# trevor-m/cuda-pathtrace

Hardware: AMD Instinct MI355X
Metric: Msamples/s, 9-sphere Cornell box 1024x1024x1024spp (higher is better)
Workload: dtype f32+f64

## Files before the change

### cuda-pathtrace_amd/__init__.py

```python
import contextlib
import ctypes
import os

import numpy as np

_HERE = os.path.dirname(os.path.abspath(__file__))
LIB_PATH = os.environ.get("PT_LIB_OVERRIDE") or os.path.join(_HERE, "libptcore.so")
LAB_LIB_PATH = os.path.join(_HERE, "libptcore_lab.so")
INCLUDE_DIR = os.path.join(os.path.dirname(_HERE), "include")

if not os.path.exists(LIB_PATH):
    raise ImportError(
        f"{LIB_PATH} is missing: build it with `make -C cuda-pathtrace_amd/csrc` "
        "(or __graft_entry__.build()); there is no fallback implementation"
    )

RNG_XORWOW = 0
RNG_PHILOX = 1
CHANNELS = 14

SPHERE_DTYPE = np.dtype([("radius", "<f4"), ("pos", "<f4", 3), ("emission", "<f4", 3), ("color", "<f4", 3)])
assert SPHERE_DTYPE.itemsize == 40


# ... 129 lines not shown
    "pt_filter_run_frames": (ctypes.c_int, [_vp, ctypes.c_int, _vp, ctypes.c_size_t, _vp, ctypes.c_size_t, ctypes.c_int, _fp]),
    "pt_temporal_opts_default": (None, [_vp]),
    "pt_temporal_create": (ctypes.c_int, [ctypes.c_int, ctypes.c_int, _vp, ctypes.POINTER(_vp)]),
    "pt_temporal_destroy": (ctypes.c_int, [_vp]),
    "pt_temporal_reset": (ctypes.c_int, [_vp]),
    "pt_temporal_workspace_bytes": (ctypes.c_int, [_vp, ctypes.POINTER(ctypes.c_uint64)]),
    "pt_temporal_camera": (ctypes.c_int, [_fp, _fp]),
    "pt_temporal_antilag_opts_default": (None, [_vp]),
    "pt_temporal_antilag_check": (ctypes.c_int, [_vp, ctypes.c_float]),
    "pt_temporal_set_antilag": (ctypes.c_int, [_vp, _vp]),
    "pt_temporal_fast": (ctypes.c_int, [_vp, _vp, _vp]),
    "pt_temporal_enqueue": (ctypes.c_int, [_vp, _vp, ctypes.c_int, _fp, _fp, _vp, _vp]),
    "pt_temporal_run": (ctypes.c_int, [_vp, _vp, ctypes.c_int, _fp, _fp, _vp, _fp]),
    "pt_temporal_enqueue_frames": (ctypes.c_int, [_vp, ctypes.c_int, _vp, ctypes.c_size_t, _fp, _fp, ctypes.c_int, _vp, _vp]),
    "pt_temporal_run_frames": (ctypes.c_int, [_vp, ctypes.c_int, _vp, ctypes.c_size_t, _fp, _fp, ctypes.c_int, _vp, _fp]),
    "pt_temporal_scene_check": (ctypes.c_int, [_vp, _vp, ctypes.c_int, _fp, _fp]),
    "pt_temporal_motion": (ctypes.c_int, [_vp, _vp, _vp, ctypes.c_int, _fp, _fp, _vp, _vp]),
    "pt_temporal_enqueue_motion": (ctypes.c_int, [_vp, _vp, ctypes.c_int, _fp, _fp, _vp, _vp, _vp]),
    "pt_temporal_run_motion": (ctypes.c_int, [_vp, _vp, ctypes.c_int, _fp, _fp, _vp, _vp, _fp]),
    "pt_temporal_enqueue_scene": (ctypes.c_int, [_vp, _vp, ctypes.c_int, _fp, _fp, _vp, ctypes.c_int, _vp, _vp]),
    "pt_temporal_run_scene": (ctypes.c_int, [_vp, _vp, ctypes.c_int, _fp, _fp, _vp, ctypes.c_int, _vp, _fp]),
    "pt_temporal_enqueue_frames_scenes": (ctypes.c_int, [_vp, ctypes.c_int, _vp, ctypes.c_size_t, _fp, _fp, _vp, ctypes.c_int, ctypes.c_int, _vp, _vp]),
    "pt_temporal_run_frames_scenes": (ctypes.c_int, [_vp, ctypes.c_int, _vp, ctypes.c_size_t, _fp, _fp, _vp, ctypes.c_int, ctypes.c_int, _vp, _fp]),
    "pt_tonemap_opts_default": (None, [_vp]),
    "pt_tonemap_create": (ctypes.c_int, [ctypes.c_int, ctypes.c_int, _vp, ctypes.POINTER(_vp)]),
    "pt_tonemap_destroy": (ctypes.c_int, [_vp]),
    "pt_tonemap_reset": (ctypes.c_int, [_vp]),
    "pt_tonemap_workspace_bytes": (ctypes.c_int, [_vp, ctypes.POINTER(ctypes.c_uint64)]),
    "pt_tonemap_reserve_frames": (ctypes.c_int, [_vp, ctypes.c_int]),
    "pt_tonemap_srgb_table": (ctypes.c_int, [_fp]),
    "pt_tonemap_enqueue": (ctypes.c_int, [_vp, _vp, ctypes.c_int, _vp, _vp]),
    "pt_tonemap_run": (ctypes.c_int, [_vp, _vp, ctypes.c_int, _vp, _fp]),
    "pt_tonemap_enqueue_frames": (ctypes.c_int, [_vp, ctypes.c_int, _vp, ctypes.c_size_t, ctypes.c_int, _vp, ctypes.c_size_t, _vp]),
    "pt_tonemap_run_frames": (ctypes.c_int, [_vp, ctypes.c_int, _vp, ctypes.c_size_t, ctypes.c_int, _vp, ctypes.c_size_t, _fp]),
    "pt_tonemap_exposure": (ctypes.c_int, [_vp, _fp]),
    "pt_compare_opts_default": (None, [_vp]),
    "pt_compare_create": (ctypes.c_int, [ctypes.c_int, ctypes.c_int, _vp, ctypes.POINTER(_vp)]),
    "pt_compare_destroy": (ctypes.c_int, [_vp]),
    "pt_compare_workspace_bytes": (ctypes.c_int, [_vp, ctypes.POINTER(ctypes.c_uint64)]),
    "pt_compare_reserve_frames": (ctypes.c_int, [_vp, ctypes.c_int]),
    "pt_compare_ssim_weights": (ctypes.c_int, [_fp]),
    "pt_compare_enqueue": (ctypes.c_int, [_vp, _vp, ctypes.c_int, _vp, ctypes.c_int, _vp, _vp]),
    "pt_compare_run": (ctypes.c_int, [_vp, _vp, ctypes.c_int, _vp, ctypes.c_int, _vp, _fp]),
    "pt_compare_enqueue_frames": (ctypes.c_int, [_vp, ctypes.c_int, _vp, ctypes.c_size_t, ctypes.c_int, _vp, ctypes.c_size_t, ctypes.c_int, _vp,
                                                 ctypes.c_size_t, _vp]),
    "pt_compare_run_frames": (ctypes.c_int, [_vp, ctypes.c_int, _vp, ctypes.c_size_t, ctypes.c_int, _vp, ctypes.c_size_t, ctypes.c_int, _vp,
                                             ctypes.c_size_t, _fp]),
    "pt_compare_result": (ctypes.c_int, [_vp, ctypes.c_int, _vp]),
    "pt_patches_opts_default": (None, [_vp]),
    "pt_patches_create": (ctypes.c_int, [ctypes.c_int, ctypes.c_int, _vp, ctypes.POINTER(_vp)]),
    "pt_patches_destroy": (ctypes.c_int, [_vp]),
    "pt_patches_workspace_bytes": (ctypes.c_int, [_vp, ctypes.POINTER(ctypes.c_uint64)]),
    "pt_patches_prepare": (ctypes.c_int, [_vp, _vp, _vp]),
    "pt_patches_score": (ctypes.c_int, [_vp, _vp, ctypes.c_int, _vp, _vp]),
    "pt_patches_result": (ctypes.c_int, [_vp, ctypes.c_int, _vp]),
    "pt_patches_gather": (ctypes.c_int, [_vp, _vp, _vp, ctypes.c_int, ctypes.c_int, _vp, _vp, _vp, _vp]),
    "pt_patches_run_prepare": (ctypes.c_int, [_vp, _vp, _fp]),
    "pt_patches_run_score": (ctypes.c_int, [_vp, _vp, ctypes.c_int, _vp, _fp]),
    "pt_patches_run_gather": (ctypes.c_int, [_vp, _vp, _vp, ctypes.c_int, ctypes.c_int, _vp, _vp, _vp, _fp]),
    "pt_progressive_create": (ctypes.c_int, [_vp, ctypes.POINTER(_vp)]),
    "pt_progressive_reset": (ctypes.c_int, [_vp]),
    "pt_progressive_enqueue": (ctypes.c_int, [_vp, ctypes.c_int, _vp, _vp, ctypes.c_int, _fp, _fp, _vp]),
    "pt_progressive_render": (ctypes.c_int, [_vp, ctypes.c_int, _vp, _vp, ctypes.c_int, _fp, _fp, _fp]),
    "pt_progressive_samples": (ctypes.c_int, [_vp, ctypes.POINTER(ctypes.c_int64)]),
    "pt_progressive_variant": (ctypes.c_int, [_vp, ctypes.c_int, ctypes.POINTER(ctypes.c_int)]),
    "pt_progressive_destroy": (ctypes.c_int, [_vp]),
    "pt_progressive_set_adaptive": (ctypes.c_int, [_vp, _vp]),
    "pt_progressive_active": (ctypes.c_int, [_vp, ctypes.POINTER(ctypes.c_int64)]),
    "pt_progressive_counts": (ctypes.c_int, [_vp, _vp, _vp]),
}
LAB_ABI = {
    "pt_debug_unary_map": (ctypes.c_int, [ctypes.c_int, _vp, _vp, ctypes.c_size_t]),
    "pt_debug_unary_compare": (ctypes.c_int, [ctypes.c_int, ctypes.c_int, ctypes.c_uint32, ctypes.c_uint64,
                                              ctypes.POINTER(ctypes.c_uint64), ctypes.POINTER(ctypes.c_uint32)]),
    "pt_debug_div_compare": (ctypes.c_int, [ctypes.c_uint32, ctypes.c_uint32, ctypes.c_uint32, ctypes.c_uint64,
                                            ctypes.POINTER(ctypes.c_uint64), ctypes.POINTER(ctypes.c_uint32),
                                            ctypes.POINTER(ctypes.c_uint32)]),
    "pt_debug_grid_header": (ctypes.c_int, [_vp, ctypes.c_int, ctypes.POINTER(ctypes.c_uint32)]),
    "pt_debug_grid_image": (ctypes.c_int, [_vp, ctypes.c_int, _fp, ctypes.c_int, ctypes.POINTER(ctypes.c_uint32), ctypes.c_size_t,
                                           ctypes.POINTER(ctypes.c_uint64)]),
    "pt_debug_policy_ms": (ctypes.c_int, [ctypes.c_int, ctypes.c_int, ctypes.c_double, ctypes.c_int, ctypes.c_int, ctypes.POINTER(ctypes.c_double)]),
    "pt_debug_policy_choice": (ctypes.c_int, [ctypes.c_int, ctypes.c_double, ctypes.c_int, ctypes.c_int, ctypes.c_int, ctypes.c_int, ctypes.POINTER(ctypes.c_int)]),
    "pt_debug_renderer_batch_launches": (ctypes.c_int, [_vp, ctypes.POINTER(ctypes.c_uint32)]),
    "pt_debug_kernel_builds": (ctypes.c_int, [ctypes.c_int, ctypes.POINTER(ctypes.c_int), ctypes.POINTER(ctypes.c_int32)]),
    "pt_debug_variant_row": (ctypes.c_int, [ctypes.c_int, ctypes.POINTER(ctypes.c_int), ctypes.POINTER(ctypes.c_int32)]),
    "pt_debug_launch_census": (ctypes.c_int, [ctypes.c_int, ctypes.POINTER(ctypes.c_uint32), ctypes.POINTER(ctypes.c_uint32)]),
    "pt_debug_launch_census_reset": (ctypes.c_int, []),
    "pt_debug_fast_nearest": (ctypes.c_int, [_vp, ctypes.c_int, _vp, ctypes.c_uint32, ctypes.c_int, ctypes.c_int, ctypes.c_uint32, _vp, _vp]),
    "pt_debug_denoiser_layer_info": (ctypes.c_int, [_vp, ctypes.c_int, ctypes.POINTER(ctypes.c_int), ctypes.POINTER(ctypes.c_int),
                                                    ctypes.c_char_p, ctypes.c_size_t]),
    "pt_debug_denoiser_activation": (ctypes.c_int, [_vp, ctypes.c_int, _vp, ctypes.c_size_t]),
    "pt_debug_denoiser_set_activation": (ctypes.c_int, [_vp, ctypes.c_int, _vp, ctypes.c_size_t]),
    "pt_debug_denoiser_conv_info": (ctypes.c_int, [_vp, ctypes.c_int, ctypes.POINTER(ctypes.c_int), ctypes.POINTER(ctypes.c_int),
                                                   ctypes.c_char_p, ctypes.c_size_t]),
    "pt_debug_denoiser_run_conv": (ctypes.c_int, [_vp, ctypes.c_int, _vp]),
    "pt_debug_denoiser_activation_frames": (ctypes.c_int, [_vp, ctypes.c_int, ctypes.c_int, _vp, ctypes.c_size_t]),
    "pt_debug_denoiser_set_activation_frames": (ctypes.c_int, [_vp, ctypes.c_int, ctypes.c_int, _vp, ctypes.c_size_t]),
    "pt_debug_denoiser_run_conv_frames": (ctypes.c_int, [_vp, ctypes.c_int, _vp, ctypes.c_int, ctypes.c_int, ctypes.c_size_t]),
    "pt_debug_denoiser_run_pre": (ctypes.c_int, [_vp, _vp, ctypes.c_int, ctypes.c_size_t, ctypes.c_int]),
    "pt_debug_denoiser_memory": (ctypes.c_int, [_vp, ctypes.c_int, ctypes.POINTER(ctypes.c_uint64)]),
    "pt_debug_denoiser_last_enqueue": (ctypes.c_int, [_vp, ctypes.POINTER(ctypes.c_int), ctypes.POINTER(ctypes.c_int)]),
    "pt_debug_denoiser_conv_plan": (ctypes.c_int, [_vp, ctypes.c_int, ctypes.c_int, ctypes.POINTER(ctypes.c_int)]),
    "pt_debug_filter_step": (ctypes.c_int, [_vp, _vp, _vp, ctypes.c_int, _vp, ctypes.c_int]),
    "pt_debug_filter_tiled": (ctypes.c_int, [_vp, ctypes.c_int]),
    "pt_debug_filter_state": (ctypes.c_int, [_vp, _vp, ctypes.c_int, _vp, ctypes.POINTER(ctypes.c_int), ctypes.c_int, _vp, _vp, _vp]),
    "pt_debug_progressive_set_samples": (ctypes.c_int, [_vp, ctypes.c_int64]),
    "pt_debug_progressive_record": (ctypes.c_int, [_vp, _vp]),
    "pt_debug_progressive_set_active": (ctypes.c_int, [_vp, _vp]),
    "pt_debug_adaptive_select": (ctypes.c_int, [_vp, ctypes.c_uint32, ctypes.c_int, ctypes.c_int, ctypes.c_int, ctypes.c_int, ctypes.c_int,
                                                ctypes.POINTER(AdaptiveOpts), _vp, _vp, _vp, _vp, _vp]),
    "pt_debug_adaptive_finalize": (ctypes.c_int, [_vp, _vp, ctypes.c_uint32, ctypes.c_int, _vp]),
}

FN_INV_SQRT_LITERAL, FN_INV_SQRT_FAST, FN_SQRT_LITERAL, FN_SQRT_FAST, FN_SIN, FN_COS, FN_UNIFORM = range(7)
FN_ONEMINUS_LITERAL, FN_ONEMINUS_FAST, FN_ONEMINUS_F32, FN_ONEMINUS_F32_FLAG, FN_ZERO = 7, 8, 9, 10, 11
FN_UNIFORM_LITERAL = 12
FN_SIN_LITERAL, FN_COS_LITERAL = 13, 14

lib = ctypes.CDLL(LIB_PATH)
for _name, (_res, _args) in ABI.items():
    if os.environ.get("PT_LIB_OVERRIDE") and not hasattr(lib, _name):
        continue
    _fn = getattr(lib, _name)
    _fn.restype = _res
    _fn.argtypes = _args
IS_LAB = hasattr(lib, "pt_debug_unary_map")
if IS_LAB:
    for _name, (_res, _args) in LAB_ABI.items():
        _fn = getattr(lib, _name)
        _fn.restype = _res
        _fn.argtypes = _args


def variants():
    out = []
    o = RendererOpts()
    for v in range(15):
        lib.pt_renderer_opts_default(ctypes.byref(o))
        o.variant = v
        h = _vp()
        rc = lib.pt_renderer_create(8, 8, 1, 8, ctypes.byref(o), ctypes.byref(h))
        if rc == 0:
            lib.pt_renderer_destroy(h)
            out.append(v)
        elif rc != -1:
            check(rc)
    return out


def build_fingerprint():
    return lib.pt_build_fingerprint().decode()


def check(rc):
    if rc != 0:
        raise PtError(rc, lib.pt_last_error().decode("utf-8", "replace"))


def _f32(a, n):
    a = np.ascontiguousarray(a, dtype=np.float32).reshape(n)
    return a, a.ctypes.data_as(_fp)


def scene_cornell():
    s = np.zeros(9, dtype=SPHERE_DTYPE)
    check(lib.pt_scene_cornell(s.ctypes.data))
# ... 278 lines not shown
        pooled.append(np.asarray(got, dtype=np.int64))
    hdr["pooled"] = pooled
    return hdr


def upload_scene(spheres):
    spheres = np.ascontiguousarray(spheres, dtype=SPHERE_DTYPE)
    return DeviceBuffer(max(spheres.nbytes, 4)).upload(spheres), len(spheres)


class Renderer(_Session):
    _destroy = "pt_renderer_destroy"

    def __init__(self, width, height, spp, threads_per_block=8, *, max_bounces=5, rng_mode=RNG_XORWOW, seed=0,
                 row_begin=0, row_end=0, persist_rng=True, variant=None, layout=LAYOUT_INTERLEAVED, fast_math=False, chunks=0):
        o = RendererOpts()
        lib.pt_renderer_opts_default(ctypes.byref(o))
        o.max_bounces, o.rng_mode, o.seed = max_bounces, rng_mode, seed
        o.row_begin, o.row_end = row_begin, row_end
        o.persist_rng = 1 if persist_rng else 0
        o.layout = layout
        o.fast_math = 1 if fast_math else 0
        o.chunks = chunks
        if variant is not None:
            o.variant = variant
        self.variant = o.variant
        h = _vp()
        check(lib.pt_renderer_create(width, height, spp, threads_per_block, ctypes.byref(o), ctypes.byref(h)))
        self.handle = h.value
        self.width, self.height, self.spp = width, height, spp
        self.row_begin = row_begin
        self.row_end = row_end if (row_begin or row_end) else height
        self.rows = self.row_end - self.row_begin

    @property
    def tile_floats(self):
        return self.rows * self.width * CHANNELS

    def render(self, d_out, d_spheres, n_spheres, basis, eye=DEFAULT_EYE):
        _, b = _f32(basis, 12)
        _, e = _f32(eye, 3)
        return self._timed(lib.pt_renderer_render, d_out, d_spheres, n_spheres, b, e)

    def enqueue(self, d_out, d_spheres, n_spheres, basis, eye=DEFAULT_EYE, stream=None):
        _, b = _f32(basis, 12)
        _, e = _f32(eye, 3)
        check(lib.pt_renderer_enqueue(self.handle, d_out, d_spheres, n_spheres, b, e, stream))

    def enqueue_frames(self, d_out, out_stride_floats, d_spheres, n_spheres, bases, eyes, d_vertices=None, vtx_stride_floats=0, stream=None):
        bases = np.ascontiguousarray(bases, dtype=np.float32).reshape(-1, 12)
        eyes = np.ascontiguousarray(eyes, dtype=np.float32).reshape(-1, 3)
        assert len(bases) == len(eyes)
        check(lib.pt_renderer_enqueue_frames(self.handle, len(bases), d_out, out_stride_floats, d_vertices, vtx_stride_floats, d_spheres,
                                             n_spheres, bases.ctypes.data_as(_fp), eyes.ctypes.data_as(_fp), stream))

    def check(self, wait=True):
        n = ctypes.c_uint32(0)
        check(lib.pt_renderer_check(self.handle, 1 if wait else 0, ctypes.byref(n)))
        return n.value

    def set_display(self, d_vertices):
        check(lib.pt_renderer_set_display(self.handle, d_vertices))

    def set_frame(self, frame):
        check(lib.pt_renderer_set_frame(self.handle, frame))

    def reset_rng(self):
        check(lib.pt_renderer_reset_rng(self.handle))

    def get_rng_state(self):
        st = np.zeros((self.rows * self.width, 6), dtype=np.uint32)
        check(lib.pt_renderer_get_rng_state(self.handle, st.ctypes.data, st.size))
        return st

    def set_rng_state(self, st):
        st = np.ascontiguousarray(st, dtype=np.uint32)
        check(lib.pt_renderer_set_rng_state(self.handle, st.ctypes.data, st.size))

    def batch_launches(self):
        n = ctypes.c_uint32(0)
        check(lib.pt_debug_renderer_batch_launches(self.handle, ctypes.byref(n)))
        return n.value

    def kernel_info(self, n_spheres):
        ki = KernelInfo()
        check(lib.pt_renderer_kernel_info(self.handle, n_spheres, ctypes.byref(ki)))
        return {f: getattr(ki, f) for f, _ in KernelInfo._fields_ if not f.startswith("reserved")}


class Progressive(_Session):
    _destroy = "pt_progressive_destroy"

    def __init__(self, renderer):
        h = _vp()
        check(lib.pt_progressive_create(renderer.handle, ctypes.byref(h)))
        self.handle = h.value
        self.renderer = renderer

    def enqueue(self, spp, d_out, d_spheres, n_spheres, basis, eye=DEFAULT_EYE, stream=None):
        _, b = _f32(basis, 12)
        _, e = _f32(eye, 3)
        check(lib.pt_progressive_enqueue(self.handle, spp, d_out, d_spheres, n_spheres, b, e, stream))

    def render(self, spp, d_out, d_spheres, n_spheres, basis, eye=DEFAULT_EYE):
        _, b = _f32(basis, 12)
        _, e = _f32(eye, 3)
        return self._timed(lib.pt_progressive_render, spp, d_out, d_spheres, n_spheres, b, e)

    def samples(self):
        n = ctypes.c_int64(0)
        check(lib.pt_progressive_samples(self.handle, ctypes.byref(n)))
        return n.value

    def reset(self):
        check(lib.pt_progressive_reset(self.handle))

    def variant(self, n_spheres):
        v = ctypes.c_int(0)
        check(lib.pt_progressive_variant(self.handle, n_spheres, ctypes.byref(v)))
        return v.value

    def set_samples(self, n):
        check(lib.pt_debug_progressive_set_samples(self.handle, n))

    def set_adaptive(self, tolerance, floor=ADAPTIVE_FLOOR, min_samples=ADAPTIVE_MIN_SAMPLES, radius=ADAPTIVE_RADIUS):
        if tolerance is None:
            check(lib.pt_progressive_set_adaptive(self.handle, None))
            return
        o = AdaptiveOpts(float(tolerance), float(floor), int(min_samples), int(radius))
        check(lib.pt_progressive_set_adaptive(self.handle, ctypes.byref(o)))

    def active(self):
        n = ctypes.c_int64(0)
        check(lib.pt_progressive_active(self.handle, ctypes.byref(n)))
        return n.value

    def counts(self):
        import torch

        n = self.renderer.rows * self.renderer.width
        t = torch.empty(n, dtype=torch.int32, device="cuda")
        if n:
            torch.cuda.synchronize()
            check(lib.pt_progressive_counts(self.handle, t.data_ptr(), None))
            torch.cuda.synchronize()
        return t

    def refine(self, max_samples, pass_spp, d_out, d_spheres, n_spheres, basis, eye=DEFAULT_EYE, on_pass=None):
        passes = 0
        while not (passes > 0 and self.active() == 0) and self.samples() + pass_spp <= max_samples:
            ms = self.render(pass_spp, d_out, d_spheres, n_spheres, basis, eye)
            if on_pass is not None:
                on_pass(self, passes, ms)
            passes += 1
        return passes

    def record(self):
        n = self.renderer.rows * self.renderer.width
        a = np.zeros((REC_WORDS, n), dtype=np.uint32)
        check(lib.pt_debug_progressive_record(self.handle, a.ctypes.data))
        return a

    def set_active(self, mask):
        m = np.ascontiguousarray(np.asarray(mask).reshape(-1) != 0, dtype=np.uint8)
        check(lib.pt_debug_progressive_set_active(self.handle, m.ctypes.data))

# ... 786 lines not shown
```

### cuda-pathtrace_amd/csrc/pt_capi.hip

```cpp
#include <hip/hip_runtime.h>
#include <math.h>

#include <climits>
#include <cstdarg>
#include <cstdio>
#include <cstdlib>
#include <cstring>
#include <new>

#include "pt_internal.h"
#include "pt_kernel.h"

namespace {
thread_local char g_err[512] = "";
}

int pt_fail(int code, const char* fmt, ...) {
  va_list ap;
  va_start(ap, fmt);
  vsnprintf(g_err, sizeof(g_err), fmt, ap);
  va_end(ap);
  return code;
}

struct pt_renderer {
  int width = 0, height = 0, spp = 0, threads_per_block = 0;
  pt_renderer_opts opts{};
  uint32_t tile_pixels = 0;
  uint32_t frame = 0;
  uint32_t* d_state = nullptr;
  hipEvent_t ev_start = nullptr, ev_stop = nullptr;
  int device = 0;
  int launch_variant = 0;
  bool auto_variant = false;
  uint64_t resident_pixels = 0;
  double waves_per_simd = 1e9;
  bool small_tile = false;
  bool spec_ok = true;
  uint32_t* d_fail = nullptr;
  uint32_t* h_fail = nullptr;
  hipEvent_t ev_fail = nullptr;
  bool fail_pending = false;
  uint32_t* d_accel = nullptr;
  uint32_t* d_chunk = nullptr;
  uint32_t chunks[PT_CHUNK_FAMILIES] = {};
  uint64_t chunk_wait_ticks = 0;
  long chunk_wait_ms = 0;
  uint32_t repaired = 0;
  float* d_vertices = nullptr;
  uint32_t* d_err = nullptr;
  uint32_t* h_err = nullptr;
  hipEvent_t ev_err = nullptr;
  bool err_pending = false;
  uint32_t debug = 0;
  uint32_t batch_launches = 0;
  hipEvent_t ev_last = nullptr;
  hipStream_t last_stream = nullptr;
  bool have_last = false;
};

static uint32_t chunks_of(const pt_renderer* r, int variant) {
  const int family = pt_kernel_variant(variant).chunk_family;
  return family == PT_CHUNK_NONE ? 0u : r->chunks[family];
}
static void chunks_off(pt_renderer* r) {
  for (uint32_t& c : r->chunks) c = 0u;
}

static const char* variant_list(char (&buf)[64], bool VariantInfo::*has, bool want = true) {
  buf[0] = 0;
  for (int v = 0, at = 0; v < pt_kernel_num_variants(); v++)
    if (pt_kernel_variant(v).*has == want) at += snprintf(buf + at, sizeof(buf) - (size_t)at, at ? ", %d" : "%d", v);
  return buf;
}

static int order_after_last(pt_renderer* r, hipStream_t stream) {
  if (r->have_last && r->last_stream != stream) PT_HIP(hipStreamWaitEvent(stream, r->ev_last, 0));
  return PT_OK;
}

static int mark_last(pt_renderer* r, hipStream_t stream) {
  PT_HIP(hipEventRecord(r->ev_last, stream));
  r->last_stream = stream;
  r->have_last = true;
  return PT_OK;
}

struct KernelCost {
  int variant, lanes;
  double L, I;
  int round;
  double unchunked, per_wave;
};
static const KernelCost kKernelCost[2][3] = {
    {{6, 1, 6.58, 2.97, 5, 1.031, 0.00666}, {8, 4, 1.85, 0.868, 5, 1.076, 0.00248}, {9, 2, 3.40, 1.60, 8, 1.108, 0.00448}},
    {{6, 1, 6.67, 3.05, 5, 1.031, 0.00666}, {8, 4, 1.75, 0.810, 8, 1.076, 0.00248}, {9, 2, 3.35, 1.60, 8, 1.108, 0.00448}}};
static const double kLaunchMs = 0.012;

static double predicted_ms(const KernelCost& c, double w, int spp, int bounces, bool chunked) {
  auto simd = [&](double k) { return c.I > 0 ? pow(pow(c.L, 4) + pow(k * c.I, 4), 0.25) : 0.0; };
  const double k = ceil(c.lanes * w - 1e-9), u = chunked ? 1.0 : c.unchunked;
  double t = simd(k);
  if (!chunked && k > c.round) {
    const double full = floor(k / c.round), rest = k - full * c.round;
    t = full * simd(c.round) + (rest > 0 ? simd(rest) : 0.0);
  }
  return kLaunchMs + k * c.per_wave + u * t * spp / 1024.0 * bounces / 5.0;
}

static int cheapest_variant(int rng_mode, double w, int spp, int bounces, bool with9, uint32_t chunked_mask) {
  int best = PT_DEFAULT_VARIANT;
  double best_ms = 1e300;
  for (const KernelCost& c : kKernelCost[rng_mode == PT_RNG_PHILOX ? 1 : 0]) {
    if (c.variant == 9 && !with9) continue;
    const double ms = predicted_ms(c, w, spp, bounces, ((chunked_mask >> c.variant) & 1u) != 0u);
    if (ms < best_ms) best = c.variant, best_ms = ms;
  }
  return best;
}

static int effective_variant(pt_renderer* r, int n_spheres) {
  if (r->opts.fast_math) return PT_VARIANT_FAST;
  if (!r->auto_variant) return r->opts.variant;
  if (r->fail_pending && hipEventQuery(r->ev_fail) == hipSuccess) {
    r->fail_pending = false;
    if (*r->h_fail > r->tile_pixels / 50u) r->spec_ok = false;
// ... 111 lines not shown
}

int pt_device_synchronize(void) {
  PT_HIP(hipDeviceSynchronize());
  return PT_OK;
}

void pt_renderer_opts_default(pt_renderer_opts* o) {
  if (!o) return;
  memset(o, 0, sizeof(*o));
  o->max_bounces = 5;
  o->rng_mode = PT_RNG_XORWOW;
  o->persist_rng = 1;
  o->variant = PT_VARIANT_AUTO;
  o->layout = PT_LAYOUT_INTERLEAVED;
  o->fast_math = 0;
  o->chunks = 0;
}

static int setup_random(pt_renderer* r) {
  if (!r->d_state) return PT_OK;
  PT_HIP(pt_launch_setup_random(r->d_state, r->width, r->opts.row_begin, r->tile_pixels, r->opts.seed, nullptr));
  PT_HIP(hipStreamSynchronize(nullptr));
  return PT_OK;
}

int pt_renderer_create(int width, int height, int samples_per_pixel, int threads_per_block,
                       const pt_renderer_opts* opts, pt_renderer** out) {
  if (!out) return pt_fail(PT_EINVAL, "pt_renderer_create: out is NULL");
  *out = nullptr;
  pt_renderer_opts o;
  if (opts) o = *opts; else pt_renderer_opts_default(&o);
  if (o.row_begin == 0 && o.row_end == 0) o.row_end = height;
  if (width <= 0 || height <= 0 || samples_per_pixel <= 0)
    return pt_fail(PT_EINVAL, "pt_renderer_create: width/height/samples must be positive (%d x %d x %d)", width, height,
                   samples_per_pixel);
  if (o.row_begin < 0 || o.row_end > height || o.row_begin > o.row_end)
    return pt_fail(PT_EINVAL, "pt_renderer_create: bad row range [%d,%d) for height %d", o.row_begin, o.row_end, height);
  if (o.max_bounces < 0 || o.max_bounces > 64) return pt_fail(PT_EINVAL, "pt_renderer_create: max_bounces %d", o.max_bounces);
  if (o.rng_mode != PT_RNG_XORWOW && o.rng_mode != PT_RNG_PHILOX)
    return pt_fail(PT_EINVAL, "pt_renderer_create: rng_mode %d", o.rng_mode);
  if (o.layout != PT_LAYOUT_INTERLEAVED && o.layout != PT_LAYOUT_PLANAR) return pt_fail(PT_EINVAL, "pt_renderer_create: layout %d", o.layout);
  if (o.fast_math != 0 && o.fast_math != 1) return pt_fail(PT_EINVAL, "pt_renderer_create: fast_math %d", o.fast_math);
  if (o.fast_math && o.variant != PT_VARIANT_AUTO)
    return pt_fail(PT_EINVAL, "pt_renderer_create: fast_math has one kernel; leave variant at -1");
  if (o.chunks < 0 || o.chunks > PT_CHUNKS_MAX || o.reserved != 0)
    return pt_fail(PT_EINVAL, "pt_renderer_create: chunks %d (0 = automatic, 1 = off, 2..%d), reserved %d (must be 0)", o.chunks, PT_CHUNKS_MAX, o.reserved);
  if (o.variant != PT_VARIANT_AUTO && !pt_kernel_has_variant(o.variant)) {
    char product[64], lab[64];
    return pt_fail(PT_EINVAL, "pt_renderer_create: kernel variant %d is not in this build (product variants: %s; the experiments %s live in libptcore_lab.so)",
                   o.variant, variant_list(product, &VariantInfo::product), variant_list(lab, &VariantInfo::product, false));
  }
  if ((uint64_t)width * (uint64_t)height > 0xFFFFFFFFull) return pt_fail(PT_EINVAL, "pt_renderer_create: image too large");

  int ndev = 0;
  PT_HIP(hipGetDeviceCount(&ndev));
  if (ndev <= 0) return pt_fail(PT_ENODEVICE, "pt_renderer_create: no HIP device");

  pt_renderer* r = new (std::nothrow) pt_renderer();
  if (!r) return pt_fail(PT_ENOMEM, "pt_renderer_create: out of host memory");
  r->width = width;
  r->height = height;
  r->spp = samples_per_pixel;
  r->threads_per_block = threads_per_block;
  r->opts = o;
  r->tile_pixels = (uint32_t)(o.row_end - o.row_begin) * (uint32_t)width;
  r->auto_variant = (o.variant == PT_VARIANT_AUTO);
  hipError_t e = hipGetDevice(&r->device);
  hipDeviceProp_t prop;
  if (e == hipSuccess) {
    e = hipGetDeviceProperties(&prop, r->device);
    if (e == hipSuccess) {
      const uint64_t simds = (uint64_t)prop.multiProcessorCount * 4u;
      r->resident_pixels = simds * 4u * 64u;
      r->waves_per_simd = (double)r->tile_pixels / (double)(simds * 64u);
      r->small_tile = (uint64_t)r->tile_pixels < simds * 64u * 3u;
    }
  }
  if (e == hipSuccess) e = hipMalloc((void**)&r->d_fail, sizeof(uint32_t));
  if (e == hipSuccess) e = hipMemset(r->d_fail, 0, sizeof(uint32_t));
  if (e == hipSuccess) e = hipHostMalloc((void**)&r->h_fail, sizeof(uint32_t), hipHostMallocDefault);
  if (e == hipSuccess) { *r->h_fail = 0; e = hipEventCreateWithFlags(&r->ev_fail, hipEventDisableTiming); }
  if (e == hipSuccess) e = hipMalloc((void**)&r->d_accel, pt_kernel_accel_bytes());
  if (e == hipSuccess) {
    set_chunk_counts(r, prop);
    int khz = 0;
    if (hipDeviceGetAttribute(&khz, hipDeviceAttributeWallClockRate, r->device) != hipSuccess || khz <= 0) khz = 100000;
    long wait_ms = 4000;
    if (const char* env = getenv("PT_CHUNK_TIMEOUT_MS")) { if (*env) wait_ms = atol(env); }
    if (wait_ms < 1) wait_ms = 1;
    r->chunk_wait_ticks = (uint64_t)khz * (uint64_t)wait_ms;
    r->chunk_wait_ms = wait_ms;
#if PT_BUILD_EXPERIMENTS
    if (const char* env = getenv("PT_LAB_DEBUG")) r->debug = (uint32_t)strtoul(env, nullptr, 0);
#endif
  }
  if (e == hipSuccess) e = hipMalloc((void**)&r->d_err, sizeof(uint32_t));
  if (e == hipSuccess) e = hipMemset(r->d_err, 0, sizeof(uint32_t));
  if (e == hipSuccess) e = hipHostMalloc((void**)&r->h_err, sizeof(uint32_t), hipHostMallocDefault);
  if (e == hipSuccess) { *r->h_err = 0; e = hipEventCreateWithFlags(&r->ev_err, hipEventDisableTiming); }
  if (e == hipSuccess) e = hipEventCreateWithFlags(&r->ev_last, hipEventDisableTiming);
  if (e == hipSuccess) e = hipEventCreate(&r->ev_start);
  if (e == hipSuccess) e = hipEventCreate(&r->ev_stop);
  if (e == hipSuccess && o.rng_mode == PT_RNG_XORWOW && o.persist_rng && r->tile_pixels)
    e = hipMalloc((void**)&r->d_state, (size_t)r->tile_pixels * 6 * sizeof(uint32_t));
  if (e != hipSuccess) {
    int rc = pt_fail(PT_EHIP, "pt_renderer_create: %s", hipGetErrorString(e));
    pt_renderer_destroy(r);
    return rc;
  }
  int rc = setup_random(r);
  if (rc != PT_OK) {
    pt_renderer_destroy(r);
    return rc;
  }
  *out = r;
  return PT_OK;
}

int pt_renderer_destroy(pt_renderer* r) {
  if (!r) return PT_OK;
  if (r->d_state) (void)hipFree(r->d_state);
  if (r->d_accel) (void)hipFree(r->d_accel);
  if (r->d_chunk) (void)hipFree(r->d_chunk);
  if (r->d_err) (void)hipFree(r->d_err);
  if (r->h_err) (void)hipHostFree(r->h_err);
  if (r->ev_err) (void)hipEventDestroy(r->ev_err);
  if (r->d_fail) (void)hipFree(r->d_fail);
  if (r->h_fail) (void)hipHostFree(r->h_fail);
  if (r->ev_fail) (void)hipEventDestroy(r->ev_fail);
  if (r->ev_last) (void)hipEventDestroy(r->ev_last);
  if (r->ev_start) (void)hipEventDestroy(r->ev_start);
  if (r->ev_stop) (void)hipEventDestroy(r->ev_stop);
  delete r;
  return PT_OK;
}

static bool chunk_buffer(pt_renderer* r, int variant, int n_spheres) {
  const uint32_t chunks = chunks_of(r, variant);
  if (chunks < 2u || !pt_kernel_chunked(variant, n_spheres, r->opts.max_bounces, r->opts.layout == PT_LAYOUT_PLANAR, r->spp, chunks))
    return false;
  if (r->d_chunk) return true;
  const size_t blocks = ((size_t)r->tile_pixels * 4 + PT_BLOCK_THREADS - 1) / PT_BLOCK_THREADS;
  if (hipMalloc((void**)&r->d_chunk, ((size_t)PT_CHUNK_WORDS * r->tile_pixels + blocks) * sizeof(uint32_t)) != hipSuccess) {
    (void)hipGetLastError();
    r->d_chunk = nullptr;
    chunks_off(r);
    return false;
  }
  return true;
}

static int take_device_error(pt_renderer* r, bool wait, uint32_t* err) {
  *err = 0u;
  if (!r->err_pending) return PT_OK;
  if (wait) PT_HIP(hipEventSynchronize(r->ev_err));
  else if (hipEventQuery(r->ev_err) != hipSuccess) { (void)hipGetLastError(); return PT_OK; }
  r->err_pending = false;
  *err = *r->h_err;
  if (*err == 0u) return PT_OK;
  *r->h_err = 0u;
  PT_HIP(hipMemset(r->d_err, 0, sizeof(uint32_t)));
  chunks_off(r);
  return PT_OK;
}

static int check_device_error(pt_renderer* r, bool wait) {
  uint32_t err = 0u;
  const int rc = take_device_error(r, wait, &err);
  if (rc != PT_OK || err == 0u) return rc;
  return pt_fail(PT_EKERNEL, "render: sample-chunk chain broken (device error word 0x%x): a workgroup waited %ld ms for its "
                             "predecessor in vain; that frame is incomplete (the pixel blocks concerned were left untouched, their "
                             "generator state included), chunking is now off for this renderer", err, r->chunk_wait_ms);
}

static int fill_args(pt_renderer* r, float* d_out, const pt_sphere* d_spheres, int n_spheres, const float basis[12],
                     const float eye[3], PixelKernelArgs* a) {
  if (!r) return pt_fail(PT_EINVAL, "render: renderer is NULL");
  if (!d_out && r->tile_pixels) return pt_fail(PT_EINVAL, "render: d_out is NULL");
  if (n_spheres < 0 || (n_spheres > 0 && !d_spheres)) return pt_fail(PT_EINVAL, "render: bad scene (%d spheres)", n_spheres);
  if (!basis || !eye) return pt_fail(PT_EINVAL, "render: basis/eye is NULL");
  const int variant = effective_variant(r, n_spheres);
  if (variant != PT_VARIANT_FAST && n_spheres > pt_kernel_max_spheres(variant))
    return pt_fail(PT_ELIMIT, "render: %d spheres exceed the LDS staging limit of %d", n_spheres,
                   pt_kernel_max_spheres(variant));
  a->fail_count = r->d_fail;
  a->accel = r->d_accel;
  a->scene_lds_f4 = 0;
  a->planar = r->opts.layout == PT_LAYOUT_PLANAR ? 1u : 0u;
  r->launch_variant = variant;
  a->out = d_out;
  a->spheres = d_spheres;
  a->rng_state = r->d_state;
  memcpy(a->basis, basis, sizeof(a->basis));
  memcpy(a->eye, eye, sizeof(a->eye));
  a->n_spheres = n_spheres;
  a->width = r->width;
  a->height = r->height;
  a->row_begin = r->opts.row_begin;
  a->tile_pixels = r->tile_pixels;
  a->spp = r->spp;
  a->max_bounces = r->opts.max_bounces;
  a->frame = r->frame;
  a->seed = r->opts.seed;
  const bool chunking = variant != PT_VARIANT_FAST && chunk_buffer(r, variant, n_spheres);
  a->chunks = chunking ? chunks_of(r, variant) : 0u;
  a->chunk_state = chunking ? r->d_chunk : nullptr;
  a->chunk_flag = chunking ? r->d_chunk + (size_t)PT_CHUNK_WORDS * r->tile_pixels : nullptr;
  a->prio = (r->spp >= 4 && (uint64_t)r->tile_pixels <= 2u * r->resident_pixels) ? 1u : 0u;
  a->err_word = r->d_err;
  a->chunk_wait_ticks = r->chunk_wait_ticks;
  a->debug = r->debug;
  a->repair = 0u;
  a->vertices = r->d_vertices;
  return PT_OK;
}

static hipError_t launch(pt_renderer* r, const PixelKernelArgs& a, hipStream_t stream) {
  if (r->launch_variant == PT_VARIANT_FAST) return pt_launch_fast_kernel(a, r->opts.rng_mode, stream);
  return pt_launch_pixel_kernel(a, r->opts.rng_mode, r->launch_variant, stream);
}

static int watch_begin(pt_renderer* r, hipStream_t stream, bool* watching) {
  *watching = r->auto_variant && pt_kernel_variant(r->launch_variant).split() && !r->fail_pending;
  if (*watching) PT_HIP(hipMemsetAsync(r->d_fail, 0, sizeof(uint32_t), stream));
  return PT_OK;
}

static int watch_error(pt_renderer* r, const PixelKernelArgs& a, hipStream_t stream) {
  if (a.chunks < 2u) return PT_OK;
  PT_HIP(hipMemcpyAsync(r->h_err, r->d_err, sizeof(uint32_t), hipMemcpyDeviceToHost, stream));
  PT_HIP(hipEventRecord(r->ev_err, stream));
  r->err_pending = true;
  return PT_OK;
}

static int watch_end(pt_renderer* r, hipStream_t stream, bool watching) {
  if (!watching) return PT_OK;
  PT_HIP(hipMemcpyAsync(r->h_fail, r->d_fail, sizeof(uint32_t), hipMemcpyDeviceToHost, stream));
  PT_HIP(hipEventRecord(r->ev_fail, stream));
  r->fail_pending = true;
  return PT_OK;
}

int pt_renderer_enqueue(pt_renderer* r, float* d_out, const pt_sphere* d_spheres, int n_spheres, const float basis[12],
                        const float eye[3], void* hip_stream) {
  PixelKernelArgs a;
  if (!r) return pt_fail(PT_EINVAL, "render: renderer is NULL");
  int rc = check_device_error(r, false);
  if (rc != PT_OK) return rc;
  rc = fill_args(r, d_out, d_spheres, n_spheres, basis, eye, &a);
  if (rc != PT_OK) return rc;
  if (r->tile_pixels == 0) return PT_OK;
  rc = order_after_last(r, (hipStream_t)hip_stream);
  if (rc != PT_OK) return rc;
  bool watching = false;
  rc = watch_begin(r, (hipStream_t)hip_stream, &watching);
  if (rc != PT_OK) return rc;
  PT_HIP(launch(r, a, (hipStream_t)hip_stream));
  rc = watch_end(r, (hipStream_t)hip_stream, watching);
  if (rc != PT_OK) return rc;
  rc = watch_error(r, a, (hipStream_t)hip_stream);
  if (rc != PT_OK) return rc;
  rc = mark_last(r, (hipStream_t)hip_stream);
  if (rc != PT_OK) return rc;
  r->frame++;
  return PT_OK;
}

int pt_renderer_enqueue_frames(pt_renderer* r, int n_frames, float* d_out, size_t out_stride_floats, float* d_vertices,
                               size_t vtx_stride_floats, const pt_sphere* d_spheres, int n_spheres, const float* bases,
                               const float* eyes, void* hip_stream) {
  if (!r) return pt_fail(PT_EINVAL, "pt_renderer_enqueue_frames: renderer is NULL");
  if (n_frames < 0 || (n_frames > 0 && (!bases || !eyes))) return pt_fail(PT_EINVAL, "pt_renderer_enqueue_frames: bad arguments");
  if (n_frames == 0) return PT_OK;
  float* const saved_vertices = r->d_vertices;
  const size_t tile_floats = (size_t)r->tile_pixels * 14u, vtx_floats = (size_t)r->tile_pixels * 3u;
  const int variant = effective_variant(r, n_spheres);
  const bool batched = n_frames >= 2 && r->tile_pixels > 0 && variant != PT_VARIANT_FAST &&
                       pt_kernel_has_frames(variant, n_spheres, r->opts.max_bounces, r->opts.layout == PT_LAYOUT_PLANAR) &&
                       (r->opts.rng_mode != PT_RNG_XORWOW || r->d_state != nullptr) &&
                       out_stride_floats >= tile_floats && (d_vertices ? vtx_stride_floats >= vtx_floats : saved_vertices == nullptr);
  int rc = PT_OK;
  for (int f0 = 0; f0 < n_frames && rc == PT_OK;) {
    const int m = batched ? (n_frames - f0 < PT_FRAMES_MAX ? n_frames - f0 : PT_FRAMES_MAX) : 1;
    float* out_f = d_out ? d_out + (size_t)f0 * out_stride_floats : nullptr;
    if (d_vertices) r->d_vertices = d_vertices + (size_t)f0 * vtx_stride_floats;
    if (m < 2) {
      rc = pt_renderer_enqueue(r, out_f, d_spheres, n_spheres, bases + 12 * (size_t)f0, eyes + 3 * (size_t)f0, hip_stream);
      f0 += 1;
      continue;
    }
    FramesKernelArgs fa;
    rc = check_device_error(r, false);
    if (rc != PT_OK) break;
    rc = fill_args(r, out_f, d_spheres, n_spheres, bases + 12 * (size_t)f0, eyes + 3 * (size_t)f0, &fa.base);
    if (rc != PT_OK) break;
    fa.base.chunks = 0u;
    fa.base.chunk_state = nullptr;
    fa.base.chunk_flag = nullptr;
    fa.frames = (uint32_t)m;
    fa.out_stride = out_stride_floats;
    fa.vtx_stride = vtx_stride_floats;
    for (int k = 0; k < m; k++) {
      memcpy(fa.cams[k], bases + 12 * (size_t)(f0 + k), 12 * sizeof(float));
      memcpy(fa.cams[k] + 12, eyes + 3 * (size_t)(f0 + k), 3 * sizeof(float));
    }
    rc = order_after_last(r, (hipStream_t)hip_stream);
    if (rc != PT_OK) break;
    {
      const hipError_t e = pt_launch_frames_kernel(fa, r->opts.rng_mode, variant, (hipStream_t)hip_stream);
      if (e != hipSuccess) { rc = pt_fail(PT_EHIP, "pt_renderer_enqueue_frames: %s", hipGetErrorString(e)); break; }
      r->batch_launches++;
    }
    rc = mark_last(r, (hipStream_t)hip_stream);
    r->frame += (uint32_t)m;
    f0 += m;
  }
  r->d_vertices = saved_vertices;
  return rc;
}

#if PT_BUILD_EXPERIMENTS
int pt_debug_renderer_batch_launches(pt_renderer* r, uint32_t* launches) {
  if (!r || !launches) return pt_fail(PT_EINVAL, "pt_debug_renderer_batch_launches: NULL argument");
  *launches = r->batch_launches;
  return PT_OK;
}
#endif

int pt_renderer_render(pt_renderer* r, float* d_out, const pt_sphere* d_spheres, int n_spheres, const float basis[12],
                       const float eye[3], float* ms_out) {
  PixelKernelArgs a;
  if (!r) return pt_fail(PT_EINVAL, "render: renderer is NULL");
  int rc = check_device_error(r, true);
  if (rc != PT_OK) return rc;
  rc = fill_args(r, d_out, d_spheres, n_spheres, basis, eye, &a);
  if (rc != PT_OK) return rc;
  if (ms_out) *ms_out = 0.0f;
  if (r->tile_pixels == 0) return PT_OK;
  rc = order_after_last(r, nullptr);
  if (rc != PT_OK) return rc;
  bool watching = false;
  rc = watch_begin(r, nullptr, &watching);
  if (rc != PT_OK) return rc;
  PT_HIP(hipEventRecord(r->ev_start, nullptr));
  PT_HIP(launch(r, a, nullptr));
  PT_HIP(hipEventRecord(r->ev_stop, nullptr));
  rc = watch_end(r, nullptr, watching);
  if (rc != PT_OK) return rc;
  rc = watch_error(r, a, nullptr);
  if (rc != PT_OK) return rc;
  PT_HIP(hipEventSynchronize(r->ev_stop));
  r->have_last = false;
  r->frame++;
  float ms = 0.0f;
  PT_HIP(hipEventElapsedTime(&ms, r->ev_start, r->ev_stop));
  uint32_t err = 0u;
  rc = take_device_error(r, true, &err);
  if (rc != PT_OK) return rc;
  if (err != 0u) {
    a.repair = a.chunks;
    a.chunks = 0u;
    PT_HIP(hipEventRecord(r->ev_start, nullptr));
    PT_HIP(launch(r, a, nullptr));
    PT_HIP(hipEventRecord(r->ev_stop, nullptr));
    PT_HIP(hipEventSynchronize(r->ev_stop));
    float ms2 = 0.0f;
    PT_HIP(hipEventElapsedTime(&ms2, r->ev_start, r->ev_stop));
    ms += ms2;
    r->repaired++;
    snprintf(g_err, sizeof(g_err), "render: sample-chunk chain broken (device error word 0x%x) -- frame repaired in place by a second, unchunked "
             "launch over the untouched pixel blocks; the returned time includes the %ld ms wait; chunking is now off for this renderer", err, r->chunk_wait_ms);
    fprintf(stderr, "ptcore: %s\n", g_err);
  }
  if (ms_out) *ms_out = ms;
  return PT_OK;
}

int pt_renderer_check(pt_renderer* r, int wait, uint32_t* repaired_frames) {
  if (!r) return pt_fail(PT_EINVAL, "pt_renderer_check: renderer is NULL");
  if (repaired_frames) *repaired_frames = r->repaired;
  return check_device_error(r, wait != 0);
}

struct pt_progressive {
  pt_renderer* r = nullptr;
  uint32_t* d_rec = nullptr;
  int64_t samples = 0;
  float cam[15] = {};
  const pt_sphere* spheres = nullptr;
  int n_spheres = 0;
  hipEvent_t ev_start = nullptr, ev_stop = nullptr;
  void* d_adaptive = nullptr;
  AdaptiveState ast{};
  AdaptiveRule rule{};
  pt_adaptive_opts opts{};
  bool forced = false;
};

static int session_variant(pt_renderer* r, int n_spheres) {
  const int v = effective_variant(r, n_spheres);
  return pt_kernel_variant(v).split() ? PT_DEFAULT_VARIANT : v;
}

int pt_progressive_create(pt_renderer* r, pt_progressive** out) {
  if (!out) return pt_fail(PT_EINVAL, "pt_progressive_create: out is NULL");
  *out = nullptr;
  if (!r) return pt_fail(PT_EINVAL, "pt_progressive_create: renderer is NULL");
  char resume[64];
  variant_list(resume, &VariantInfo::resume);
// ... 12 lines not shown
    pt_progressive_destroy(p);
    return rc;
  }
  *out = p;
  return PT_OK;
}

int pt_progressive_destroy(pt_progressive* p) {
  if (!p) return PT_OK;
  if (p->d_rec) (void)hipFree(p->d_rec);
  if (p->d_adaptive) (void)hipFree(p->d_adaptive);
  if (p->ev_start) (void)hipEventDestroy(p->ev_start);
  if (p->ev_stop) (void)hipEventDestroy(p->ev_stop);
  delete p;
  return PT_OK;
}

int pt_progressive_reset(pt_progressive* p) {
  if (!p) return pt_fail(PT_EINVAL, "pt_progressive_reset: session is NULL");
  p->samples = 0;
  p->forced = false;
  return PT_OK;
}

static int session_sync(const pt_progressive* p) {
  if (p->r->have_last) PT_HIP(hipEventSynchronize(p->r->ev_last));
  return PT_OK;
}

int pt_progressive_samples(const pt_progressive* p, int64_t* samples) {
  if (!p || !samples) return pt_fail(PT_EINVAL, "pt_progressive_samples: NULL argument");
  *samples = p->samples;
  if (p->d_adaptive && p->samples > 0 && p->r->tile_pixels) {
    int rc = session_sync(p);
    if (rc != PT_OK) return rc;
    uint32_t w = 0u;
    PT_HIP(hipMemcpy(&w, p->ast.words + 1, sizeof(w), hipMemcpyDeviceToHost));
    *samples = (int64_t)w;
  }
  return PT_OK;
}

int pt_progressive_variant(const pt_progressive* p, int n_spheres, int* variant) {
  if (!p || !variant) return pt_fail(PT_EINVAL, "pt_progressive_variant: NULL argument");
  *variant = session_variant(p->r, n_spheres);
  return PT_OK;
}

static int progressive_args(pt_progressive* p, int spp, float* d_out, const pt_sphere* d_spheres, int n_spheres, const float basis[12],
                            const float eye[3], ResumeKernelArgs* ra, int* variant) {
  if (!p) return pt_fail(PT_EINVAL, "pt_progressive: session is NULL");
  pt_renderer* r = p->r;
  if (spp < 1) return pt_fail(PT_EINVAL, "pt_progressive: spp %d (a pass adds at least one sample)", spp);
  if (!d_out && r->tile_pixels) return pt_fail(PT_EINVAL, "pt_progressive: d_out is NULL");
  if (n_spheres < 0 || (n_spheres > 0 && !d_spheres)) return pt_fail(PT_EINVAL, "pt_progressive: bad scene (%d spheres)", n_spheres);
  if (!basis || !eye) return pt_fail(PT_EINVAL, "pt_progressive: basis/eye is NULL");
  if ((int64_t)spp > (int64_t)INT_MAX - p->samples)
    return pt_fail(PT_EINVAL, "pt_progressive: %lld + %d samples exceed INT_MAX (the reference's counts are int)", (long long)p->samples, spp);
  if (p->samples > 0 && (memcmp(p->cam, basis, 12 * sizeof(float)) != 0 || memcmp(p->cam + 12, eye, 3 * sizeof(float)) != 0 ||
                         p->spheres != d_spheres || p->n_spheres != n_spheres))
    return pt_fail(PT_EINVAL, "pt_progressive: camera or scene differs from the session's first pass: reset the session");
  const int v = session_variant(r, n_spheres);
  if (!pt_kernel_has_resume(v)) return pt_fail(PT_EINVAL, "pt_progressive: kernel variant %d has no progressive passes", v);
  if (n_spheres > pt_kernel_max_spheres(v))
    return pt_fail(PT_ELIMIT, "pt_progressive: %d spheres exceed the LDS staging limit of %d", n_spheres, pt_kernel_max_spheres(v));
  *variant = v;
  PixelKernelArgs& a = ra->base;
  memset(&a, 0, sizeof(a));
  a.out = d_out;
  a.spheres = d_spheres;
  a.rng_state = nullptr;
  memcpy(a.basis, basis, sizeof(a.basis));
  memcpy(a.eye, eye, sizeof(a.eye));
  a.n_spheres = n_spheres;
  a.width = r->width;
  a.height = r->height;
  a.row_begin = r->opts.row_begin;
  a.tile_pixels = r->tile_pixels;
  a.spp = (int32_t)(p->samples + spp);
  a.max_bounces = r->opts.max_bounces;
  a.frame = 0u;
  a.planar = r->opts.layout == PT_LAYOUT_PLANAR ? 1u : 0u;
  a.fail_count = nullptr;
  a.accel = r->d_accel;
  a.seed = r->opts.seed;
  a.err_word = r->d_err;
  a.chunk_wait_ticks = r->chunk_wait_ticks;
  a.debug = r->debug;
  a.vertices = nullptr;
  a.prio = (spp >= 4 && (uint64_t)r->tile_pixels <= 2u * r->resident_pixels) ? 1u : 0u;
  ra->sample_begin = (int32_t)p->samples;
  ra->session = p->d_rec;
  return PT_OK;
}

static void progressive_advance(pt_progressive* p, int spp, const pt_sphere* d_spheres, int n_spheres, const float basis[12], const float eye[3]) {
  if (p->samples == 0) {
    memcpy(p->cam, basis, 12 * sizeof(float));
    memcpy(p->cam + 12, eye, 3 * sizeof(float));
    p->spheres = d_spheres;
    p->n_spheres = n_spheres;
  }
  p->samples += spp;
}

static int launch_progressive_pass(pt_progressive* p, const ResumeKernelArgs& ra, int variant, hipStream_t stream) {
  pt_renderer* r = p->r;
  if (!p->d_adaptive) {
    PT_HIP(pt_launch_resume_kernel(ra, r->opts.rng_mode, variant, stream));
    return PT_OK;
  }
  const int mode = p->forced ? 1 : (p->samples == 0 ? 2 : 0);
  PT_HIP(pt_launch_adaptive_select(p->ast, p->rule, p->d_rec, r->tile_pixels, r->width, (int)p->samples, ra.base.spp, mode, false, stream));
  AdaptiveKernelArgs aa;
  static_cast<ResumeKernelArgs&>(aa) = ra;
  aa.list = p->ast.list;
  aa.list_len = p->ast.words;
  PT_HIP(pt_launch_adaptive_kernel(aa, r->opts.rng_mode, variant, stream));
  PT_HIP(pt_launch_adaptive_finalize(p->d_rec, p->ast.counts, ra.base.out, r->tile_pixels, r->opts.layout == PT_LAYOUT_PLANAR, stream));
  p->forced = false;
  return PT_OK;
}

int pt_progressive_enqueue(pt_progressive* p, int spp, float* d_out, const pt_sphere* d_spheres, int n_spheres, const float basis[12],
                           const float eye[3], void* hip_stream) {
  ResumeKernelArgs ra;
  int variant = 0;
  int rc = progressive_args(p, spp, d_out, d_spheres, n_spheres, basis, eye, &ra, &variant);
  if (rc != PT_OK) return rc;
  pt_renderer* r = p->r;
  if (r->tile_pixels) {
    const hipStream_t stream = (hipStream_t)hip_stream;
    rc = order_after_last(r, stream);
    if (rc != PT_OK) return rc;
    rc = launch_progressive_pass(p, ra, variant, stream);
    if (rc != PT_OK) return rc;
    rc = mark_last(r, stream);
    if (rc != PT_OK) return rc;
  }
  progressive_advance(p, spp, d_spheres, n_spheres, basis, eye);
  return PT_OK;
}

int pt_progressive_render(pt_progressive* p, int spp, float* d_out, const pt_sphere* d_spheres, int n_spheres, const float basis[12],
                          const float eye[3], float* ms_out) {
  ResumeKernelArgs ra;
  int variant = 0;
  if (ms_out) *ms_out = 0.0f;
  int rc = progressive_args(p, spp, d_out, d_spheres, n_spheres, basis, eye, &ra, &variant);
  if (rc != PT_OK) return rc;
  pt_renderer* r = p->r;
  if (r->tile_pixels) {
    rc = order_after_last(r, nullptr);
    if (rc != PT_OK) return rc;
    PT_HIP(hipEventRecord(p->ev_start, nullptr));
    rc = launch_progressive_pass(p, ra, variant, nullptr);
    if (rc != PT_OK) return rc;
    PT_HIP(hipEventRecord(p->ev_stop, nullptr));
    PT_HIP(hipEventSynchronize(p->ev_stop));
    r->have_last = false;
    float ms = 0.0f;
    PT_HIP(hipEventElapsedTime(&ms, p->ev_start, p->ev_stop));
    if (ms_out) *ms_out = ms;
  }
  progressive_advance(p, spp, d_spheres, n_spheres, basis, eye);
  return PT_OK;
}
// ... 193 lines not shown
```

### cuda-pathtrace_amd/csrc/pt_intersect.h

```cpp
#pragma once
#include "pt_scene_lds.h"

#pragma clang fp contract(off)

namespace pt {

template <int LEVEL>
__device__ __forceinline__ bool intersect_scene_loop(const SceneLds& sc, int n, F3 o, F3 d, const RayConst& rc,
                                                     float& t_hit, int& idx) {
  float tNearest = 1000000.0f;
  float t = 0.0f;
  bool hit = false;
#pragma clang loop unroll(disable)
  for (int i = 0; i < n; i++) {
    const float4 g = sc.geom_uniform(i);
    bool h;
    if constexpr (LEVEL == 0)
      h = intersect_sphere(o, d, rc.a, g, t);
    else
      h = intersect_sphere_v1(o, d, rc, g, t);
    if (h && t > 0.0f && t < tNearest) {
      tNearest = t;
      hit = true;
      t_hit = t;
// ... 51 lines not shown
    }
  }
  if (__builtin_expect(ambiguous, 0)) hit = intersect_scene_loop<1>(sc, n, o, d, rc, t_hit, idx);
  return hit;
}

__device__ __forceinline__ void screen_tail(float b, float a4c, float det, float dacc, float num, float TA, float TB,
                                            float Tlim_hi, int i, float& T1, float& T2, int& i1, bool& unsure) {
  const float INF = __builtin_inff();
  const float lo = fminf(TA, TB), hi = fmaxf(TA, TB);
  const float T = lo > 0.0f ? lo : hi;
  const bool real = (det >= 0.0f) & (dacc >= 0.0f);
  const bool ok = real & (T > 0.0f) & (T < Tlim_hi);
  unsure = unsure | (real & !((fabsf(num) > fabsf(a4c) * 4.7683716e-07f) & (fabsf(T) < INF)));
  const float Te = ok ? T : INF;
  const bool c1 = Te < T1, c2 = Te < T2;
  T2 = c1 ? T1 : (c2 ? Te : T2);
  i1 = c1 ? i : i1;
  T1 = c1 ? Te : T1;
  (void)b;
}

__device__ __forceinline__ bool intersect_scene_screened_pk(const SceneLds& sc, int n, F3 o, F3 d, const RayConst& rc,
                                                            float& t_hit, int& idx) {
  const float INF = __builtin_inff();
  const float Tlim = 1000000.0f * (2.0f * rc.a);
  const float Tlim_hi = Tlim * 1.0000153f;
  float T1 = INF, T2 = INF;
  int i1 = 0;
  bool unsure = false;
  const v2f ox = {o.x, o.x}, oy = {o.y, o.y}, oz = {o.z, o.z};
  const v2f dx = {d.x, d.x}, dy = {d.y, d.y}, dz = {d.z, d.z};
  const v2f a4 = {rc.a4, rc.a4};
  const int npairs = (n + 1) >> 1;
  for (int p = 0; p < npairs; p++) {
    const float4 A = sc.pair[2 * p], B = sc.pair[2 * p + 1];
    const v2f offx = ox - v2f{A.x, A.y}, offy = oy - v2f{A.z, A.w}, offz = oz - v2f{B.x, B.y};
    const v2f dd = dx * offx + dy * offy + dz * offz;
    const v2f b = dd + dd;
    const v2f c = (offx * offx + offy * offy + offz * offz) - v2f{B.z, B.w};
    const v2f bb = b * b;
    const v2f a4c = a4 * c;
    const v2f det = bb - a4c;
    const v2f dacc = __builtin_elementwise_fma(-a4, c, bb);
    const v2f e = __builtin_elementwise_fma(b, b, -bb);
    const v2f num = a4c + e;
    const v2f s = {__builtin_amdgcn_sqrtf(fmaxf(dacc.x, 0.0f)), __builtin_amdgcn_sqrtf(fmaxf(dacc.y, 0.0f))};
    const v2f q = b + v2f{copysignf(s.x, b.x), copysignf(s.y, b.y)};
    const v2f r = {__builtin_amdgcn_rcpf(q.x), __builtin_amdgcn_rcpf(q.y)};
    const v2f TA = -q;
    const v2f TB = -num * r;
    screen_tail(b.x, a4c.x, det.x, dacc.x, num.x, TA.x, TB.x, Tlim_hi, 2 * p, T1, T2, i1, unsure);
    screen_tail(b.y, a4c.y, det.y, dacc.y, num.y, TA.y, TB.y, Tlim_hi, 2 * p + 1, T1, T2, i1, unsure);
  }
  bool ambiguous = unsure | ((T1 < INF) & ((T2 <= T1 * 1.0000038f) | (T1 >= Tlim * 0.99998f)));
  bool hit = false;
  if (!ambiguous && T1 < INF) {
    float t;
    if (intersect_sphere_v1(o, d, rc, sc.geom[i1], t) && t > 0.0f && t < 1000000.0f) {
      hit = true;
      t_hit = t;
      idx = i1;
    } else {
      ambiguous = true;
    }
  }
  if (__builtin_expect(ambiguous, 0)) hit = intersect_scene_loop<1>(sc, n, o, d, rc, t_hit, idx);
  return hit;
}

__device__ __forceinline__ uint32_t umed3(uint32_t a, uint32_t b, uint32_t c) {
  uint32_t r;
  asm("v_med3_u32 %0, %1, %2, %3" : "=v"(r) : "v"(a), "v"(b), "v"(c));
  return r;
}

struct ScreenState {
  uint32_t k1, k2;
  bool unsure;
  uint32_t absmask;
};

__device__ __forceinline__ uint32_t screen_sphere_oc(F3 off, float c, int i, F3 d, const RayConst& rc, uint32_t imask, ScreenState& st);
__device__ __forceinline__ uint32_t screen_sphere(const float4 g, int i, F3 o, F3 d, const RayConst& rc, uint32_t imask,
                                                  ScreenState& st) {
  const F3 off = mk3(o.x - g.x, o.y - g.y, o.z - g.z);
  return screen_sphere_oc(off, dot(off, off) - g.w, i, d, rc, imask, st);
}
__device__ __forceinline__ void screen_insert(ScreenState& st, uint32_t key) {
  st.k2 = umed3(st.k1, st.k2, key);
  st.k1 = st.k1 < key ? st.k1 : key;
}
template <class F>
__device__ __forceinline__ void screen_nine(ScreenState& st, F key_of) {
  auto umin = [](uint32_t x, uint32_t y) { return x < y ? x : y; };
  auto umax = [](uint32_t x, uint32_t y) { return x > y ? x : y; };
  uint32_t lead[3], next[3];
#pragma unroll
  for (int g3 = 0; g3 < 3; g3++) {
    const uint32_t x = key_of(3 * g3), y = key_of(3 * g3 + 1), z = key_of(3 * g3 + 2);
    lead[g3] = umin(umin(x, y), z);
    next[g3] = umed3(x, y, z);
  }
  const uint32_t l = umin(lead[0], lead[1]);
  const uint32_t r2 = umin(umin(umax(lead[0], lead[1]), next[0]), next[1]);
  st.k1 = umin(l, lead[2]);
  st.k2 = umin(umin(umax(l, lead[2]), r2), next[2]);
}
__device__ __forceinline__ uint32_t screen_sphere_oc(F3 off, float c, int i, F3 d, const RayConst& rc, uint32_t imask, ScreenState& st) {
  const float h = dot(d, off);
  const float hh = h * h;
  const float ac = rc.a * c;
  const float dacc = fmaf(-rc.a, c, hh);
  const float s = __builtin_amdgcn_sqrtf(dacc);
  const float e = fmaf(h, h, -hh);
  const float num = ac + e;
  const float TA = copysign_neg_b3(s, h, st.absmask) - h;
  const float TB = num * __builtin_amdgcn_rcpf(TA);
  const uint32_t ta = __float_as_uint(TA), tb = __float_as_uint(TB);
  const uint32_t tbits = ta < tb ? ta : tb;
  const uint32_t key = bitop3<0xBA>(tbits, imask, (uint32_t)i);
#ifndef PT_MUTANT_NO_DOUBT
  st.unsure = st.unsure | !(fabsf(ac) > fmaf(hh, 1.1920929e-07f, 1e-30f));
#endif
  return key;
}

__device__ __forceinline__ bool neg_finite(float x) { return __builtin_amdgcn_classf(x, 0x18); }
template <int AX>
__device__ __forceinline__ F3 with_axis(F3 v, float x) {
  return mk3(AX == 0 ? x : v.x, AX == 1 ? x : v.y, AX == 2 ? x : v.z);
}
template <int AX>
__device__ __forceinline__ uint32_t screen_wall_pair(const uint4 t, uint32_t m, F3 o, F3 d, const RayConst& rc, uint32_t imask,
                                                     ScreenState& st, float& hb, bool& inb) {
  const float4 gf = lds_read_f4(bitop3<0xE4>(t.y, t.x, m)), gb = lds_read_f4(bitop3<0xE4>(t.x, t.y, m));
  const F3 off = mk3(o.x - gf.x, o.y - gf.y, o.z - gf.z);
  const F3 sq = off * off, pr = d * off;
  const float ob = AX == 0 ? o.x - gb.x : AX == 1 ? o.y - gb.y : o.z - gb.z;
  const F3 sqb = with_axis<AX>(sq, ob * ob), prb = with_axis<AX>(pr, (AX == 0 ? d.x : AX == 1 ? d.y : d.z) * ob);
  hb = (prb.x + prb.y) + prb.z;
  inb = neg_finite(fmaf(gb.w, 5.9837103e-08f, ((sqb.x + sqb.y) + sqb.z) - gb.w));
  return screen_sphere_oc(off, ((sq.x + sq.y) + sq.z) - gf.w, (int)bitop3<0xE4>(t.w, t.z, m), d, rc, imask, st);
}
template <bool WALLS>
__device__ __forceinline__ void screen_walled(ScreenState& st, const uint4* W, F3 o, F3 d, const RayConst& rc, uint32_t imask,
                                              uint32_t lim_hi_bits) {
  auto umin = [](uint32_t x, uint32_t y) { return x < y ? x : y; };
  auto umax = [](uint32_t x, uint32_t y) { return x > y ? x : y; };
  const float4* Wg = reinterpret_cast<const float4*>(W);
  const uint4 oi = W[3];
  auto sel = [](uint32_t dbits) { return (uint32_t)((int32_t)dbits >> 31); };
  const uint32_t mx = sel(__float_as_uint(d.x)), my = sel(__float_as_uint(d.y)), mz = sel(__float_as_uint(d.z));
  const uint32_t a0 = screen_sphere(Wg[0], (int)oi.x, o, d, rc, imask, st), a1 = screen_sphere(Wg[1], (int)oi.y, o, d, rc, imask, st),
                 a2 = screen_sphere(Wg[2], (int)oi.z, o, d, rc, imask, st);
  const uint32_t l0 = umin(umin(a0, a1), a2), n0 = umed3(a0, a1, a2);
  float h0, h1, h2;
  bool in0, in1, in2;
  if constexpr (WALLS) __builtin_amdgcn_sched_barrier(0);
  const uint32_t b0 = screen_wall_pair<0>(W[4], mx, o, d, rc, imask, st, h0, in0);
  if constexpr (WALLS) __builtin_amdgcn_sched_barrier(0);
  const uint32_t b1 = screen_wall_pair<1>(W[5], my, o, d, rc, imask, st, h1, in1);
  if constexpr (WALLS) __builtin_amdgcn_sched_barrier(0);
  const uint32_t b2 = screen_wall_pair<2>(W[6], mz, o, d, rc, imask, st, h2, in2);
  if constexpr (WALLS) __builtin_amdgcn_sched_barrier(0);
  const uint32_t l1 = umin(umin(b0, b1), b2), n1 = umed3(b0, b1, b2);
  st.k1 = umin(l0, l1);
  st.k2 = umin(umin(umax(l0, l1), n0), n1);
  const float K = __uint_as_float(st.k1 & ~imask) * __uint_as_float(oi.w);
  const bool cert = (st.k1 < lim_hi_bits) & (neg_finite(fmaf(2.0f, h0, K)) & in0) & (neg_finite(fmaf(2.0f, h1, K)) & in1) &
                    (neg_finite(fmaf(2.0f, h2, K)) & in2);
  if (__builtin_expect(__builtin_amdgcn_ballot_w64(!cert) != 0, 0)) {
    auto behind = [&](int k, uint32_t m) {
      const uint4 t = W[4 + k];
      screen_insert(st, screen_sphere(lds_read_f4(bitop3<0xE4>(t.x, t.y, m)), (int)bitop3<0xE4>(t.z, t.w, m), o, d, rc, imask, st));
    };
    behind(0, mx);
    behind(1, my);
    behind(2, mz);
  }
}

#ifdef PT_SCREEN_STATS
__device__ unsigned long long g_screen_stats[8];
#endif
template <bool NB, bool PRIMARY = false, bool LAST = false, bool WALLS = false>
__device__ __forceinline__ bool intersect_scene_screened_keys(const SceneLds& sc, int n, F3 o, F3 d, const RayConst& rc,
                                                              float& t_hit, int& idx) {
  if (n <= 0) return false;
  const float Tlim = 1000000.0f * rc.a;
  const uint32_t lim_hi_bits = __float_as_uint(Tlim * 1.0000153f);
  const int ib = 32 - __builtin_clz((unsigned)(n > 1 ? n - 1 : 1));
  const uint32_t imask = (1u << ib) - 1u;
  const float margin = 1.0f + (__builtin_ldexpf(1.0f, ib - 22) + 7.6293945e-06f);
  ScreenState st{0xFFFFFFFFu, 0xFFFFFFFFu, false, sc.absmask};
  auto key_of = [&](const float4 g, int i) -> uint32_t {
    if constexpr (PRIMARY) {
      const float4 e = sc.eyeg[i];
      return screen_sphere_oc(mk3(e.x, e.y, e.z), e.w, i, d, rc, imask, st);
    } else {
      return screen_sphere(g, i, o, d, rc, imask, st);
    }
  };
  auto screen = [&](const float4 g, int i) { screen_insert(st, key_of(g, i)); };
  int i = 0;
  if constexpr (PRIMARY) {
    const uint32_t full = n >= 32 ? 0xFFFFFFFFu : (1u << n) - 1u;
    uint32_t m = __builtin_amdgcn_readfirstlane(sc.prim_mask) & full;
    if (m != full) {
      while (m) {
        const int j = __builtin_ctz(m);
        m &= m - 1u;
        screen(sc.geom[j], j);
      }
      i = n;
    }
  }
#if PT_UNROLL_NINE
  if constexpr (!PRIMARY) {
    if (sc.walls && n == 9) {
      screen_walled<WALLS>(st, sc.walls, o, d, rc, imask, lim_hi_bits);
      i = 9;
    }
  }
  if (i == 0 && n == 9) {
    screen_nine(st, [&](int u) { return key_of(sc.geom[u], u); });
    i = 9;
  }
#endif
  for (; i + 3 <= n; i += 3) {
    const float4 g0 = sc.geom[i], g1 = sc.geom[i + 1], g2 = sc.geom[i + 2];
    screen(g0, i);
    screen(g1, i + 1);
    screen(g2, i + 2);
  }
  for (; i < n; i++) screen(sc.geom[i], i);
  const uint32_t k1 = st.k1, k2 = st.k2;
  const bool has = k1 < lim_hi_bits;
  const float T1 = __uint_as_float(k1 & ~imask);
  bool ambiguous = st.unsure | (has & (((k2 & ~imask) <= __float_as_uint(T1 * margin)) | (T1 >= Tlim * 0.99998f)));
  bool hit = false;
  if constexpr (NB && LAST && !PRIMARY) {
    const int i1 = (int)(k1 & imask);
    const float4 g = sc.geom[has ? i1 : 0];
    const F3 off = mk3(o.x - g.x, o.y - g.y, o.z - g.z);
    const float h = dot(d, off);
    const float c = dot(off, off) - g.w;
    const float ac = rc.a * c;
    const float dacc = fmaf(-rc.a, c, h * h);
    const bool certain = (dacc > fabsf(ac) * 4.7683716e-07f) & (T1 >= rc.a * 1e-30f);
    ambiguous = ambiguous | (has & !certain);
    hit = has;
    t_hit = T1;
    idx = i1;
    if (__builtin_expect(ambiguous, 0)) hit = intersect_scene_loop<0>(sc, n, o, d, rc, t_hit, idx);
    return hit;
  } else if constexpr (NB) {
    const int i1 = (int)(k1 & imask);
    float t;
    bool bad = false;
    bool real;
    if constexpr (PRIMARY) {
      const float4 e = sc.eyeg[has ? i1 : 0];
      real = intersect_sphere_nb_oc(mk3(e.x, e.y, e.z), e.w, d, rc, t, bad);
    } else {
      real = intersect_sphere_nb(o, d, rc, sc.geom[has ? i1 : 0], t, bad);
    }
    const bool good = real & (t >= kMinGoodT) & (t < 1000000.0f);
#ifdef PT_SCREEN_STATS
    {
      const bool tie = has & ((k2 & ~imask) <= __float_as_uint(T1 * margin));
      const bool lim = has & (T1 >= Tlim * 0.99998f);
      const uint64_t any = __builtin_amdgcn_ballot_w64(ambiguous | (has & (bad | !good)));
      if ((threadIdx.x & 63) == __builtin_ctzll(__builtin_amdgcn_ballot_w64(true))) {
        atomicAdd(&g_screen_stats[0], 1ull);
        atomicAdd(&g_screen_stats[1], any != 0 ? 1ull : 0ull);
      }
      atomicAdd(&g_screen_stats[2], (ambiguous | (has & (bad | !good))) ? 1ull : 0ull);
      atomicAdd(&g_screen_stats[3], st.unsure ? 1ull : 0ull);
      atomicAdd(&g_screen_stats[4], tie ? 1ull : 0ull);
      atomicAdd(&g_screen_stats[5], lim ? 1ull : 0ull);
      atomicAdd(&g_screen_stats[6], (has & bad) ? 1ull : 0ull);
      atomicAdd(&g_screen_stats[7], (has & !good) ? 1ull : 0ull);
    }
#endif
    ambiguous = ambiguous | (has & (bad | !good));
    hit = has & good;
    t_hit = t;
    idx = i1;
#ifdef PT_TIMING_ONLY_DETECT_NO_REDO
    if (__builtin_expect(ambiguous, 0)) hit = false;
#elif !defined(PT_TIMING_ONLY_NO_ISECT_REDO)
    if (__builtin_expect(ambiguous, 0)) hit = intersect_scene_loop<0>(sc, n, o, d, rc, t_hit, idx);
#endif
    return hit;
  } else {
    if (!ambiguous && has) {
      const int i1 = (int)(k1 & imask);
      float t;
      if (intersect_sphere_v1(o, d, rc, sc.geom[i1], t) && t > 0.0f && t < 1000000.0f) {
        hit = true;
        t_hit = t;
        idx = i1;
      } else {
// ... 230 lines not shown
```

### cuda-pathtrace_amd/csrc/pt_kernel.h

```cpp
#pragma once
#include <hip/hip_runtime.h>
#include <stddef.h>
#include <stdint.h>

#include "../../include/ptcore.h"

#ifndef PT_BLOCK_THREADS
#define PT_BLOCK_THREADS 256
#endif
#ifndef PT_PRIO_MIN_SPP
#define PT_PRIO_MIN_SPP 512
#endif
#ifndef PT_PRIO_MIN_SPP_REGEN
#define PT_PRIO_MIN_SPP_REGEN 32
#endif
#ifndef PT_FOOTPRINT_MIN_SPP
#define PT_FOOTPRINT_MIN_SPP 8
#endif
#ifndef PT_SCREEN_UNROLL
#define PT_SCREEN_UNROLL 9
#endif
#define PT_VARIANT_AUTO (-1)
#define PT_DEFAULT_VARIANT 6
#ifndef PT_SCREEN_MAX_SPHERES
// ... 42 lines not shown
#define PT_V13_WELFORD_TABLE 1
#endif
#ifndef PT_V13_DEAD_END
#define PT_V13_DEAD_END 1
#endif
#ifndef PT_POOL_MIN_WAVES
#define PT_POOL_MIN_WAVES 4
#endif
#define PT_GRID_MAX_SPHERES 2048
#define PT_GRID_MIN_SPHERES 160
#ifndef PT_GRID_MIN_SPHERES_LARGE_TILE
#define PT_GRID_MIN_SPHERES_LARGE_TILE 72
#endif

struct PixelKernelArgs {
  float* out;
  const pt_sphere* spheres;
  uint32_t* rng_state;
  float basis[12];
  float eye[3];
  int32_t n_spheres;
  int32_t width, height;
  int32_t row_begin;
  uint32_t tile_pixels;
  int32_t spp;
  int32_t max_bounces;
  uint32_t frame;
  uint32_t scene_lds_f4;
  uint32_t planar;
  uint32_t* fail_count;
  const uint32_t* accel;
  uint64_t seed;
  uint32_t chunks;
  uint32_t* chunk_state;
  uint32_t* chunk_flag;
  uint32_t* err_word;
  uint64_t chunk_wait_ticks;
  uint32_t debug;
  uint32_t prio;
  float* vertices;
  uint32_t repair;
};
#define PT_FRAMES_MAX 32
struct FramesKernelArgs {
  PixelKernelArgs base;
  uint32_t frames;
  uint64_t out_stride;
  uint64_t vtx_stride;
  float cams[PT_FRAMES_MAX][15];
};
struct ResumeKernelArgs {
  PixelKernelArgs base;
  int32_t sample_begin;
  uint32_t* session;
};
struct AdaptiveKernelArgs : ResumeKernelArgs {
  const uint32_t* list;
  const uint32_t* list_len;
};
#define PT_CHUNK_WORDS 26
enum {
  PT_REC_COLOR = 0, PT_REC_NORMAL = 3, PT_REC_ALBEDO = 6,
  PT_REC_DEPTH = 9,
  PT_REC_N_COLOR = 10, PT_REC_N_HIT = 11,
  PT_REC_MEAN = 12, PT_REC_M2 = 13,
  PT_REC_RNG = 20,
};
static_assert(PT_REC_RNG + 6 == PT_CHUNK_WORDS && PT_REC_MEAN + 2 * 4 == PT_REC_RNG, "the record's layout");
#ifndef PT_CHUNKS
#define PT_CHUNKS 2
#endif
#define PT_CHUNKS_TILE 8
#define PT_CHUNKS_SMALL_TILE 6
#define PT_CHUNKS_SPLIT 4
#define PT_CHUNKS_MAX 16
#ifndef PT_CHUNKS_GRID_MAX
#define PT_CHUNKS_GRID_MAX 4
#endif
#define PT_CHUNK_MAX_SAMPLES 4096
#define PT_CHUNK_MAX_SAMPLES_GRID 256
#define PT_DEVERR_CHUNK_CHAIN 1u
#define PT_CHUNK_FAILED 0x80000000u
#define PT_DEBUG_DROP_CHUNK_FLAG 1u

#ifndef PT_BUILD_EXPERIMENTS
#define PT_BUILD_EXPERIMENTS 0
#endif
#define PT_VARIANT_FAST 100
#define PT_FAST_LDS_SPHERES 64
enum { PT_LEAN_NEVER, PT_LEAN_BIG, PT_LEAN_ALWAYS };
enum { PT_LDS_PLAIN, PT_LDS_PACKED, PT_LDS_WALLS };
enum { PT_GRID_NONE, PT_GRID_LANE, PT_GRID_POOLED };
enum { PT_CHUNK_NONE = -1, PT_CHUNK_ONE_LANE, PT_CHUNK_SPLIT, PT_CHUNK_GRID, PT_CHUNK_FAMILIES };
enum { PT_LOOP_SAMPLES, PT_LOOP_PAIRS, PT_LOOP_REGEN, PT_LOOP_DECOUPLED };
struct VariantInfo {
  bool product;
  int lanes;
  int threads;
  int lean;
  int lds_extra;
  int grid;
  bool wide;
  bool ref_builds;
  bool resume;
  bool frames;
  int chunk_family;
  bool can_chunk;
  int min_waves;
  int loop;
  int tracer;
  int kernel;
  constexpr bool split() const { return lanes > 1; }
  constexpr bool chunk_build(bool ref) const { return can_chunk && (!ref_builds || ref); }
};
const VariantInfo& pt_kernel_variant(int variant);
int pt_kernel_num_variants(void);
bool pt_kernel_chunked(int variant, int n_spheres, int max_bounces, bool planar, int spp, uint32_t chunks);
int pt_kernel_ref_bounces(int n_spheres, int max_bounces, int variant, bool planar);
int pt_kernel_block_threads(int variant);
bool pt_kernel_has_variant(int variant);
const void* pt_kernel_symbol(int rng_mode, int variant, int n_spheres, int max_bounces, bool planar);
size_t pt_kernel_lds_bytes(int n_spheres, int variant);
int pt_kernel_max_spheres(int variant);
hipError_t pt_launch_pixel_kernel(const PixelKernelArgs& a, int rng_mode, int variant, hipStream_t stream);
bool pt_kernel_has_frames(int variant, int n_spheres, int max_bounces, bool planar);
hipError_t pt_launch_frames_kernel(const FramesKernelArgs& fa, int rng_mode, int variant, hipStream_t stream);
bool pt_kernel_has_resume(int variant);
const void* pt_resume_kernel_symbol(int rng_mode, int variant, int n_spheres, int max_bounces, bool planar);
hipError_t pt_launch_resume_kernel(const ResumeKernelArgs& ra, int rng_mode, int variant, hipStream_t stream);
const void* pt_adaptive_kernel_symbol(int rng_mode, int variant, int n_spheres, int max_bounces, bool planar);
hipError_t pt_launch_adaptive_kernel(const AdaptiveKernelArgs& aa, int rng_mode, int variant, hipStream_t stream);
struct AdaptiveState {
  uint32_t* counts;
  uint32_t* list;
  uint8_t* mask;
  uint32_t* block_sums;
  uint32_t* words;
};
struct AdaptiveRule {
  double tolerance;
  double floor;
  int32_t min_samples;
  int32_t radius;
};
inline AdaptiveRule pt_adaptive_rule(const pt_adaptive_opts& o) {
  return AdaptiveRule{(double)o.tolerance, (double)o.floor, o.min_samples, o.radius};
}
#define PT_ADAPTIVE_BLOCK 256
#define PT_ADAPTIVE_MAX_RADIUS 4
hipError_t pt_launch_adaptive_select(const AdaptiveState& s, const AdaptiveRule& rule, const uint32_t* rec, uint32_t tile_pixels,
                                     int width, int n, int n_end, int mode, bool peek, hipStream_t stream);
hipError_t pt_launch_adaptive_finalize(const uint32_t* rec, const uint32_t* counts, float* out, uint32_t tile_pixels, bool planar,
                                       hipStream_t stream);
hipError_t pt_launch_build_grid(const pt_sphere* spheres, int n, uint32_t* accel, const float* eye ,
                                bool pooled , hipStream_t stream,
                                int threads = PT_GRID_BLOCK_THREADS );
void pt_kernel_grid_layout(int n_spheres, int threads, uint64_t out[8]);
size_t pt_kernel_accel_bytes(void);
hipError_t pt_launch_setup_random(uint32_t* state, int width, int row_begin, uint32_t tile_pixels, uint64_t seed,
                                  hipStream_t stream);
const void* pt_fast_kernel_symbol(int rng_mode, int n_spheres, int max_bounces);
size_t pt_fast_kernel_lds_bytes(int n_spheres);
hipError_t pt_launch_fast_kernel(const PixelKernelArgs& a, int rng_mode, hipStream_t stream);

#if PT_BUILD_EXPERIMENTS
#include "../../include/ptcore_lab.h"
hipError_t pt_census_launched(const void* fn, uint32_t modes);
#define PT_LAUNCHED(fn, modes) pt_census_launched((const void*)(fn), (modes))
#else
#define PT_LAUNCHED(fn, modes) hipGetLastError()
#endif
```

### cuda-pathtrace_amd/csrc/pt_kernel.hip

```cpp
#include "pt_trace.h"

#pragma clang fp contract(off)

static constexpr int kNumVariants = 15;
static constexpr int kT = PT_BLOCK_THREADS, kTG = PT_GRID_BLOCK_THREADS, kTW = PT_GRID_WIDE_THREADS;
static constexpr int kW = PT_MIN_WAVES, kWG = PT_GRID_MIN_WAVES, kWD = PT_GRID12_MIN_WAVES, kWP = PT_POOL_MIN_WAVES;
static constexpr VariantInfo kVariants[kNumVariants] = {
     {true,  1, kT,  PT_LEAN_NEVER,  PT_LDS_PLAIN,  PT_GRID_NONE,   false, false, false, false, PT_CHUNK_NONE,     false, kW,   PT_LOOP_SAMPLES,   0,     0},
     {false, 1, kT,  PT_LEAN_NEVER,  PT_LDS_PLAIN,  PT_GRID_NONE,   false, false, false, false, PT_CHUNK_NONE,     false, kW,   PT_LOOP_SAMPLES,   1,     1},
     {false, 1, kT,  PT_LEAN_NEVER,  PT_LDS_PLAIN,  PT_GRID_NONE,   false, false, false, false, PT_CHUNK_NONE,     false, kW,   PT_LOOP_SAMPLES,   2,     2},
     {false, 1, kT,  PT_LEAN_NEVER,  PT_LDS_PACKED, PT_GRID_NONE,   false, false, false, false, PT_CHUNK_NONE,     false, kW,   PT_LOOP_SAMPLES,   3,     3},
     {false, 1, kT,  PT_LEAN_NEVER,  PT_LDS_PLAIN,  PT_GRID_NONE,   false, false, false, false, PT_CHUNK_NONE,     false, kW,   PT_LOOP_SAMPLES,   4,     4},
     {false, 1, kT,  PT_LEAN_NEVER,  PT_LDS_PLAIN,  PT_GRID_NONE,   false, false, false, false, PT_CHUNK_NONE,     false, kW,   PT_LOOP_SAMPLES,   5,     5},
     {true,  1, kT,  PT_LEAN_BIG,    PT_LDS_WALLS,  PT_GRID_NONE,   false, true,  true,  true,  PT_CHUNK_ONE_LANE, true,  kW,   PT_LOOP_SAMPLES,   6,     6},
     {false, 1, kT,  PT_LEAN_NEVER,  PT_LDS_PLAIN,  PT_GRID_NONE,   false, false, false, false, PT_CHUNK_NONE,     false, kW,   PT_LOOP_PAIRS,     6,     7},
     {true,  4, kT,  PT_LEAN_BIG,    PT_LDS_PLAIN,  PT_GRID_NONE,   false, true,  false, false, PT_CHUNK_SPLIT,    true,  0,    PT_LOOP_SAMPLES,   6,     8},
     {true,  2, kT,  PT_LEAN_NEVER,  PT_LDS_PLAIN,  PT_GRID_NONE,   false, true,  false, false, PT_CHUNK_SPLIT,    true,  0,    PT_LOOP_SAMPLES,   6,     9},
     {true,  1, kT,  PT_LEAN_BIG,    PT_LDS_PLAIN,  PT_GRID_NONE,   false, false, true,  false, PT_CHUNK_NONE,     false, kW,   PT_LOOP_REGEN,     6,     10},
     {false, 1, kTG, PT_LEAN_ALWAYS, PT_LDS_PLAIN,  PT_GRID_LANE,   false, false, false, false, PT_CHUNK_NONE,     false, kWG,  PT_LOOP_REGEN,     11,    11},
     {false, 1, kTG, PT_LEAN_ALWAYS, PT_LDS_PLAIN,  PT_GRID_LANE,   false, false, false, false, PT_CHUNK_NONE,     false, kWD,  PT_LOOP_DECOUPLED, 11,    12},
     {true,  1, kTG, PT_LEAN_ALWAYS, PT_LDS_PLAIN,  PT_GRID_POOLED, false, false, true,  false, PT_CHUNK_GRID,     true,  kWP,  PT_LOOP_REGEN,     13,    13},
     {true,  1, kTW, PT_LEAN_ALWAYS, PT_LDS_PLAIN,  PT_GRID_POOLED, true,  false, true,  false, PT_CHUNK_GRID,     false, kWP,  PT_LOOP_REGEN,     13,    13},
};
static constexpr VariantInfo kNoVariant = {false, 1, kT, PT_LEAN_NEVER, PT_LDS_PLAIN, PT_GRID_NONE, false, false, false, false, PT_CHUNK_NONE, false, kW, PT_LOOP_SAMPLES, 0, 0};

template <class P>
constexpr bool every_row(P holds) {
  for (int i = 0; i < kNumVariants; i++)
    if (!holds(i, kVariants[i], kVariants[kVariants[i].kernel])) return false;
  return true;
}
static_assert(every_row([](int, const VariantInfo& r, const VariantInfo&) { return r.kernel >= 0 && r.kernel < kNumVariants; }), "every row's kernel is a row");
static_assert(every_row([](int i, const VariantInfo& r, const VariantInfo& k) { return (r.wide || r.kernel == i) && !k.wide; }), "only a wide row runs another row's kernel");
static_assert(every_row([](int, const VariantInfo& r, const VariantInfo& k) { return !r.wide || (k.grid == PT_GRID_POOLED && r.threads == kTW); }), "a wide row names a pooled-grid kernel");
static_assert(every_row([](int, const VariantInfo& r, const VariantInfo& k) { return (!r.resume || k.resume) && (!r.frames || k.frames) && (!r.ref_builds || k.ref_builds); }),
              "a row's resume, frames and reference-configuration builds are its kernel's");
static_assert(every_row([](int, const VariantInfo& r, const VariantInfo& k) {
                return r.lean == k.lean && r.lds_extra == k.lds_extra && r.grid == k.grid && r.min_waves == k.min_waves && r.loop == k.loop && r.tracer == k.tracer;
              }), "a wide row differs from its kernel's in the workgroup only");
static_assert(every_row([](int, const VariantInfo& r, const VariantInfo&) { return !r.frames || (r.lanes == 1 && r.ref_builds); }), "frames builds: one-lane rows, reference configurations");
static_assert(every_row([](int, const VariantInfo& r, const VariantInfo&) { return !r.split() || (!r.resume && !r.wide && r.grid == PT_GRID_NONE); }), "pixel_kernel_split: no resume, wide or grid builds");
constexpr int split_row(int lanes) {
  for (int i = 0; i < kNumVariants; i++)
    if (kVariants[i].split() && kVariants[i].lanes == lanes) return i;
  return -1;
}
constexpr int launch_row(int kernel, bool wide) {
  for (int i = 0; wide && i < kNumVariants; i++)
    if (kVariants[i].wide && kVariants[i].kernel == kernel) return i;
  return wide ? -1 : kernel;
}

namespace pt {

template <int VAR, bool WIDE = false>
constexpr int kBlockThreads = kVariants[launch_row(VAR, WIDE)].threads;

template <int VAR, int REFB, int RNG>
constexpr int kMinWavesR = (kVariants[VAR].ref_builds && REFB != 0) ? (RNG == PT_RNG_XORWOW ? PT_REF_MIN_WAVES : (REFB == 5 ? PT_REF_MIN_WAVES_PHILOX : kVariants[VAR].min_waves))
                                                                      : kVariants[VAR].min_waves;

__device__ __forceinline__ bool chunk_wait(const PixelKernelArgs& a, uint32_t block_id, uint32_t chunk) {
  __shared__ uint32_t s_pred;
  if (threadIdx.x == 0) {
    const uint64_t t0 = wall_clock64();
    uint32_t spins = 0, f;
    for (;;) {
      f = __hip_atomic_load(a.chunk_flag + block_id, __ATOMIC_ACQUIRE, __HIP_MEMORY_SCOPE_AGENT);
      if ((f & PT_CHUNK_FAILED) != 0u || f >= chunk) break;
      __builtin_amdgcn_s_sleep(32);
      if ((++spins & 255u) == 0u && wall_clock64() - t0 > a.chunk_wait_ticks) {
        f = PT_CHUNK_FAILED;
        break;
      }
    }
    if ((f & PT_CHUNK_FAILED) != 0u) {
      if (a.err_word) atomicOr(a.err_word, PT_DEVERR_CHUNK_CHAIN);
      __hip_atomic_fetch_or(a.chunk_flag + block_id, PT_CHUNK_FAILED, __ATOMIC_RELEASE, __HIP_MEMORY_SCOPE_AGENT);
    }
    s_pred = f;
  }
  __syncthreads();
  return (s_pred & PT_CHUNK_FAILED) != 0u;
}

__device__ __forceinline__ void chunk_publish(const PixelKernelArgs& a, uint32_t block_id, uint32_t chunk) {
  __syncthreads();
  if (threadIdx.x == 0) {
    __threadfence();
#if PT_BUILD_EXPERIMENTS
    if ((a.debug & PT_DEBUG_DROP_CHUNK_FLAG) && block_id == 0u && chunk == 0u) return;
#endif
    __hip_atomic_fetch_max(a.chunk_flag + block_id, chunk + 1u, __ATOMIC_RELEASE, __HIP_MEMORY_SCOPE_AGENT);
  }
}

template <bool FRAMES, bool RESUME = false, bool ADAPTIVE = false> struct KernelArgsOf { typedef PixelKernelArgs type; };
template <> struct KernelArgsOf<true, false, false> { typedef FramesKernelArgs type; };
template <> struct KernelArgsOf<false, true, false> { typedef ResumeKernelArgs type; };
template <> struct KernelArgsOf<false, true, true> { typedef AdaptiveKernelArgs type; };
template <bool FRAMES, bool RESUME, bool ADAPTIVE> __device__ __forceinline__ PixelKernelArgs& base_args(typename KernelArgsOf<FRAMES, RESUME, ADAPTIVE>::type& args) {
  if constexpr (FRAMES || RESUME) return args.base; else return args;
}

template <int RNG, int VAR, bool LEAN = false, int REFB = 0, bool FRAMES = false, bool WIDE = false, bool RESUME = false, bool ADAPTIVE = false>
__global__ void __launch_bounds__((kBlockThreads<VAR, WIDE>), (((FRAMES || (RESUME && REFB == 8)) && RNG == PT_RNG_XORWOW) ? PT_MIN_WAVES : kMinWavesR<VAR, REFB, RNG>)) PT_KERNEL_ATTR
pixel_kernel(typename KernelArgsOf<FRAMES, RESUME, ADAPTIVE>::type args) {
  PixelKernelArgs& a = base_args<FRAMES, RESUME, ADAPTIVE>(args);
  constexpr VariantInfo K = kVariants[VAR];
  constexpr bool POOLED = K.grid == PT_GRID_POOLED;
  static_assert(K.kernel == VAR && !K.split() && kVariants[launch_row(VAR, WIDE)].wide == WIDE, "a pixel_kernel build is a one-lane row's own kernel, WIDE a wide row's");
  static_assert(!ADAPTIVE || RESUME, "adaptive passes are resume builds");
  uint32_t n_active = 0u;
  if constexpr (ADAPTIVE) {
    n_active = __builtin_amdgcn_readfirstlane(*args.list_len);
    if (blockIdx.x * (uint32_t)kBlockThreads<VAR, WIDE> >= n_active) return;
  }
  constexpr bool FRAME_GRID = FRAMES && RNG == PT_RNG_PHILOX, FRAME_LOOP = FRAMES && !FRAME_GRID;
  uint32_t fr = 0u, fr_count = 1u, first_block = blockIdx.x;
  auto load_camera = [&](uint32_t f) {
    if constexpr (FRAMES) {
      typedef const __attribute__((address_space(4))) float* cfloats;
      typedef const __attribute__((address_space(4))) char* cbytes;
      const cfloats cam = (cfloats)((cbytes)__builtin_amdgcn_kernarg_segment_ptr() + offsetof(FramesKernelArgs, cams)) + 15u * f;
#pragma unroll
      for (int k = 0; k < 12; k++) a.basis[k] = cam[k];
#pragma unroll
      for (int k = 0; k < 3; k++) a.eye[k] = cam[12 + k];
    }
  };
  if constexpr (FRAMES) fr_count = args.frames;
  if constexpr (FRAME_GRID) {
    const uint32_t n_blocks = (a.tile_pixels + kBlockThreads<VAR, WIDE> - 1) / kBlockThreads<VAR, WIDE>;
    fr = blockIdx.x / n_blocks;
    first_block = blockIdx.x - fr * n_blocks;
    load_camera(fr);
  }
  constexpr bool REF = REFB != 0;
  constexpr bool CHUNKS = K.chunk_build(REF) && !FRAMES && !RESUME;
  static_assert(!REF || K.ref_builds, "reference-configuration builds: the rows that announce them");
  static_assert(!LEAN ? K.lean != PT_LEAN_ALWAYS : K.lean != PT_LEAN_NEVER, "the LDS layouts of the row");
  static_assert(!FRAMES || (K.frames && REF), "frame batches: reference-configuration builds of the rows with frames (variant 6)");
  static_assert(!RESUME || (!FRAMES && K.resume), "progressive passes: the rows with resume (variants 6, 10, 13; 14 = WIDE)");
  int sample_begin = 0;
  if constexpr (RESUME) sample_begin = args.sample_begin;
  const int pass_spp = a.spp - sample_begin;
  if constexpr (REF) {
    a.n_spheres = 9;
    a.max_bounces = REFB;
  }
  if constexpr (CHUNKS) {
    if (a.repair != 0u && __hip_atomic_load(a.chunk_flag + blockIdx.x, __ATOMIC_RELAXED, __HIP_MEMORY_SCOPE_AGENT) == a.repair) return;
  }
  extern __shared__ float4 lds_scene[];
  SceneLds sc = stage_scene<K.lds_extra == PT_LDS_PACKED>(a.spheres, a.n_spheres, lds_scene, LEAN, mk3(a.eye[0], a.eye[1], a.eye[2]), a.spp);
  sc.small_only = !LEAN && K.lean == PT_LEAN_BIG;
  constexpr bool kWalls = K.lds_extra == PT_LDS_WALLS && REFB == 5 && !LEAN;
  if constexpr (kWalls) stage_walls(sc, a.spheres, a.n_spheres);
  constexpr bool kRegen = K.loop == PT_LOOP_REGEN, kDecoupled = K.loop == PT_LOOP_DECOUPLED;
  GridLds grid;
  if constexpr (K.grid != PT_GRID_NONE) {
    grid = stage_grid<POOLED>(a.spheres, a.n_spheres, a.accel, lds_scene + a.scene_lds_f4);
    sc.grid = &grid;
    if constexpr (POOLED)
      sc.pool = reinterpret_cast<char*>(lds_scene + a.scene_lds_f4) + ((grid_lds_bytes(a.n_spheres, true, kBlockThreads<VAR, WIDE>) + 15) & ~(size_t)15);
  }

  uint32_t block_id = FRAMES ? first_block : blockIdx.x, chunk = 0u, n_chunks = 1u;
  if constexpr (CHUNKS) {
    if (a.chunks > 1u) {
      const uint32_t n_blocks = (a.tile_pixels + kBlockThreads<VAR, WIDE> - 1) / kBlockThreads<VAR, WIDE>;
      n_chunks = a.chunks;
      chunk = blockIdx.x / n_blocks;
      block_id = blockIdx.x - chunk * n_blocks;
    }
  }
  const uint32_t slot = block_id * kBlockThreads<VAR, WIDE> + threadIdx.x;
  const bool active = ADAPTIVE ? slot < n_active : slot < a.tile_pixels;
  const uint32_t tp = [&]() -> uint32_t {
    if constexpr (ADAPTIVE) return active ? args.list[slot] : 0u; else return slot;
  }();
  const int row = a.row_begin + (int)(tp / (uint32_t)a.width);
  const int col = (int)(tp % (uint32_t)a.width);
  const uint32_t id = (uint32_t)row * (uint32_t)a.width + (uint32_t)col;

  Rng<RNG> rng;
  if constexpr (RNG == PT_RNG_XORWOW) {
    if (a.rng_state && active) {
      const uint32_t* s = a.rng_state + (size_t)tp * 6;
      rng.st = Xorwow{s[0], s[1], s[2], s[3], s[4], s[5]};
    } else {
      xorwow_init(rng.st, (uint64_t)id + a.seed);
    }
  } else {
    rng.k0 = (uint32_t)a.seed;
    rng.k1 = (uint32_t)(a.seed >> 32) ^ a.frame;
    rng.pix = id;
  }

  const bool pow2_image = ((a.width & (a.width - 1)) == 0) && ((a.height & (a.height - 1)) == 0);
  const float inv_w = 1.0f / (float)a.width, inv_h = 1.0f / (float)a.height;

frame_top:
  if constexpr (FRAME_LOOP) {
    load_camera(fr);
    if (fr > 0u) {
      __syncthreads();
      for (int i = threadIdx.x; i < a.n_spheres; i += blockDim.x) {
        const float4 g = sc.geom[i];
        const F3 off = mk3(a.eye[0] - g.x, a.eye[1] - g.y, a.eye[2] - g.z);
        sc.eyeg[i] = make_float4(off.x, off.y, off.z, dot(off, off) - g.w);
      }
      __syncthreads();
    }
  }
  if constexpr (FRAMES && RNG == PT_RNG_PHILOX) rng.k1 = (uint32_t)(a.seed >> 32) ^ (a.frame + fr);
  const F3 B0 = mk3(a.basis[0], a.basis[1], a.basis[2]), B1 = mk3(a.basis[3], a.basis[4], a.basis[5]);
  const F3 B2 = mk3(a.basis[6], a.basis[7], a.basis[8]), B3 = mk3(a.basis[9], a.basis[10], a.basis[11]);
  const F3 eye = mk3(a.eye[0], a.eye[1], a.eye[2]);

  Welford var[4] = {{0, 0.0f, 0.0f}, {0, 0.0f, 0.0f}, {0, 0.0f, 0.0f}, {0, 0.0f, 0.0f}};
  TraceOutput L{mk3(0, 0, 0), mk3(0, 0, 0), mk3(0, 0, 0), 0.0f};
  int i_begin = sample_begin, i_end = a.spp;
  if constexpr (RESUME) {
    if (sample_begin > 0 && active) {
      const uint32_t* rec = args.session;
      auto ld = [&](int w) { return rec[(size_t)w * a.tile_pixels + tp]; };
      auto ldf = [&](int w) { return __uint_as_float(ld(w)); };
      L.color = mk3(ldf(PT_REC_COLOR), ldf(PT_REC_COLOR + 1), ldf(PT_REC_COLOR + 2));
      L.normal = mk3(ldf(PT_REC_NORMAL), ldf(PT_REC_NORMAL + 1), ldf(PT_REC_NORMAL + 2));
      L.albedo = mk3(ldf(PT_REC_ALBEDO), ldf(PT_REC_ALBEDO + 1), ldf(PT_REC_ALBEDO + 2));
      L.depth = ldf(PT_REC_DEPTH);
      const int n0 = (int)ld(PT_REC_N_COLOR), n1 = (int)ld(PT_REC_N_HIT);
#pragma unroll
      for (int k = 0; k < 4; k++) var[k] = Welford{k == 0 ? n0 : n1, ldf(PT_REC_MEAN + 2 * k), ldf(PT_REC_M2 + 2 * k)};
      if constexpr (RNG == PT_RNG_XORWOW) rng.st = Xorwow{ld(PT_REC_RNG), ld(PT_REC_RNG + 1), ld(PT_REC_RNG + 2), ld(PT_REC_RNG + 3), ld(PT_REC_RNG + 4), ld(PT_REC_RNG + 5)};
    }
  }
  if constexpr (CHUNKS) {
    if (n_chunks > 1u) {
      const int per = (a.spp + (int)n_chunks - 1) / (int)n_chunks;
// ... 137 lines not shown
    GridWalk w;
    w.a = 1.0f;
    w.s = Near2{0.0f, 0.0f, 0};
    w.tmax0 = w.tmax1 = w.tmax2 = w.tdel0 = w.tdel1 = w.tdel2 = 0.0f;
    w.cidx = w.cs0 = w.cs1 = w.cs2 = 0;
    w.left = w.k0 = w.k1 = w.n0 = w.n1 = 0u;
    w.have_next = w.walking = w.forced = false;
    w.e0 = w.e1 = 0u;
    w.t_box = 0.0f;
    bool in_walk = false;
    bool brute = false;
    for (;;) {
      if (__builtin_amdgcn_ballot_w64(i < a.spp) == 0) break;
      const bool ready = (i < a.spp) & !(in_walk & !brute & w.busy());
      if (ready) {
        if (in_walk) {
          float t = 0.0f;
          int idx = 0;
          bool hit = false;
          if (a.n_spheres > 0) {
            if (brute) hit = intersect_scene_screened_large(sc, a.n_spheres, o, d, make_ray_const(d), t, idx);
            else hit = grid_end(w, sc, grid, a.n_spheres, o, d, t, idx);
          }
          const bool escaped = !bounce_shade<RNG, K.tracer>(L, sc, o, d, color, mask, rng, var, n, hit, t, idx);
          n++;
          if (escaped | (n >= a.max_bounces)) {
            if (!escaped) {
              L.color = L.color + color;
              if (sc.lean) welford_update(var[0], luminance(color)); else welford_update(var[0], luminance(color), sc.rcpn);
            }
            i++;
            n = 0;
          }
          in_walk = false;
        }
        if (i < a.spp) {
          if (n == 0) {
            rng.begin_sample((uint32_t)i);
            primary_ray(rng, d);
            o = eye;
            color = mk3(0.0f, 0.0f, 0.0f);
            mask = mk3(1.0f, 1.0f, 1.0f);
          }
          const float aa = dot(d, d);
          brute = !(grid.valid && a.n_spheres > 0 && grid_admits(grid, o, d, aa));
          if (!brute) grid_begin(w, grid, o, d, aa);
          in_walk = true;
        }
      }
      grid_trips<true>(w, grid, o, d, in_walk & !brute, i < a.spp, PT_GRID_PARK);
    }
  }
  if constexpr (K.loop == PT_LOOP_PAIRS) {
    const int draws = (a.spp != 1 ? 2 : 0) + 2 * a.max_bounces;
    for (; i + 2 <= a.spp; i += 2) {
      Rng<RNG> g[2] = {rng, rng};
      g[0].begin_sample((uint32_t)i);
      if constexpr (RNG == PT_RNG_XORWOW) xorwow_skip(g[1].st, draws);
      g[1].begin_sample((uint32_t)i + 1u);
      F3 o2[2] = {eye, eye}, d2[2];
      primary_ray(g[0], d2[0]);
      primary_ray(g[1], d2[1]);
      PathResult res[2];
      trace_paths<RNG, 2>(res, sc, a.n_spheres, o2, d2, g, a.max_bounces);
      accumulate_path(L, var, res[0]);
      if (RNG == PT_RNG_XORWOW && __builtin_expect(res[0].escaped, 0)) {
        rng = g[0];
        rng.begin_sample((uint32_t)i + 1u);
        F3 dir;
        primary_ray(rng, dir);
        trace_ray<RNG, K.tracer>(L, sc, a.n_spheres, eye, dir, rng, var, a.max_bounces);
      } else {
        accumulate_path(L, var, res[1]);
        rng = g[1];
      }
    }
  }
  if constexpr (!kRegen && !kDecoupled) {
    const int span = i_end - i_begin;
    const bool by_progress = a.prio != 0u && span >= 4;
    const int q1 = i_begin + span / 4, q2 = i_begin + span / 2, q3 = i_end - span / 4;
    const int stride_mask = span >= 64 ? 15 : 0;
    const int i_stop = active ? i_end : i;
    for (; i < i_stop; i++) {
      if (by_progress) {
        const int iu = __builtin_amdgcn_readfirstlane(i);
        if ((iu & stride_mask) == 0) {
          if (iu < q1) __builtin_amdgcn_s_setprio(3);
          else if (iu < q2) __builtin_amdgcn_s_setprio(2);
          else if (iu < q3) __builtin_amdgcn_s_setprio(1);
          else __builtin_amdgcn_s_setprio(0);
        }
      }
      rng.begin_sample((uint32_t)i);
      F3 dir;
      primary_ray(rng, dir);
      trace_ray<RNG, K.tracer, REFB, kWalls>(L, sc, a.n_spheres, eye, dir, rng, var, a.max_bounces);
    }
    if (by_progress) __builtin_amdgcn_s_setprio(0);
  }
  if constexpr (CHUNKS) {
    if (chunk + 1u < n_chunks) {
      if (active) {
        auto st = [&](int w, uint32_t v) { a.chunk_state[(size_t)w * a.tile_pixels + tp] = v; };
        auto stf = [&](int w, float v) { st(w, __float_as_uint(v)); };
        stf(PT_REC_COLOR, L.color.x); stf(PT_REC_COLOR + 1, L.color.y); stf(PT_REC_COLOR + 2, L.color.z);
        stf(PT_REC_NORMAL, L.normal.x); stf(PT_REC_NORMAL + 1, L.normal.y); stf(PT_REC_NORMAL + 2, L.normal.z);
        stf(PT_REC_ALBEDO, L.albedo.x); stf(PT_REC_ALBEDO + 1, L.albedo.y); stf(PT_REC_ALBEDO + 2, L.albedo.z);
        stf(PT_REC_DEPTH, L.depth);
        st(PT_REC_N_COLOR, (uint32_t)var[0].n);
        st(PT_REC_N_HIT, (uint32_t)var[1].n);
#pragma unroll
        for (int k = 0; k < 4; k++) {
          stf(PT_REC_MEAN + 2 * k, var[k].mean);
          stf(PT_REC_M2 + 2 * k, var[k].M2);
        }
        if constexpr (RNG == PT_RNG_XORWOW) {
          st(PT_REC_RNG, rng.st.d); st(PT_REC_RNG + 1, rng.st.v0); st(PT_REC_RNG + 2, rng.st.v1); st(PT_REC_RNG + 3, rng.st.v2); st(PT_REC_RNG + 4, rng.st.v3); st(PT_REC_RNG + 5, rng.st.v4);
        }
      }
      chunk_publish(a, block_id, chunk);
      return;
    }
  }

  const float fs = (float)a.spp;
  float px[14];
  frame_values(L, var, fs, px);
  float* out_f = a.out;
  float* vtx_f = a.vertices;
  if constexpr (FRAMES) {
    out_f += (size_t)fr * args.out_stride;
    if (vtx_f) vtx_f += (size_t)fr * args.vtx_stride;
  }
  if (!ADAPTIVE && vtx_f && active) store_display_vertex(vtx_f + (size_t)tp * 3, a.width, row, col, px[0], px[1], px[2]);
  if (ADAPTIVE) {
  } else if (!REF && a.planar) {
    if (active) {
#pragma unroll
      for (int c = 0; c < 14; c++) out_f[(size_t)c * a.tile_pixels + tp] = px[c];
    }
  } else {
  const int lane = threadIdx.x & 63, wave = threadIdx.x >> 6;
  const bool wave_full = (__builtin_amdgcn_ballot_w64(active) == ~0ull) && ((reinterpret_cast<uintptr_t>(out_f) & 15u) == 0u) &&
                         K.grid == PT_GRID_NONE;
  if (wave_full) {
    float* wl = reinterpret_cast<float*>(lds_scene + a.scene_lds_f4) + wave * (64 * 14);
#pragma unroll
    for (int c = 0; c < 14; c++) wl[lane * 14 + c] = px[c];
    __builtin_amdgcn_wave_barrier();
    const float4* src = reinterpret_cast<const float4*>(wl);
    float4* dst = reinterpret_cast<float4*>(out_f + (size_t)(tp - (uint32_t)lane) * 14);
#pragma unroll
    for (int k = 0; k < 4; k++) {
      const int q = lane + 64 * k;
      if (q < 224) dst[q] = src[q];
    }
  } else if (active) {
    float* o = out_f + (size_t)tp * 14;
#pragma unroll
    for (int c = 0; c < 14; c++) o[c] = px[c];
  }
  }
  if constexpr (FRAME_LOOP) {
    __builtin_amdgcn_wave_barrier();
    if (++fr < fr_count) goto frame_top;
  }
  if constexpr (RESUME) {
    if (active) {
      uint32_t* rec = args.session;
      auto st = [&](int w, uint32_t v) { rec[(size_t)w * a.tile_pixels + tp] = v; };
      auto stf = [&](int w, float v) { st(w, __float_as_uint(v)); };
      stf(PT_REC_COLOR, L.color.x); stf(PT_REC_COLOR + 1, L.color.y); stf(PT_REC_COLOR + 2, L.color.z);
      stf(PT_REC_NORMAL, L.normal.x); stf(PT_REC_NORMAL + 1, L.normal.y); stf(PT_REC_NORMAL + 2, L.normal.z);
      stf(PT_REC_ALBEDO, L.albedo.x); stf(PT_REC_ALBEDO + 1, L.albedo.y); stf(PT_REC_ALBEDO + 2, L.albedo.z);
      stf(PT_REC_DEPTH, L.depth);
      st(PT_REC_N_COLOR, (uint32_t)var[0].n);
      st(PT_REC_N_HIT, (uint32_t)var[1].n);
#pragma unroll
      for (int k = 0; k < 4; k++) {
// ... 276 lines not shown
    } else {
      base += 1;
      if constexpr (RNG == PT_RNG_XORWOW) rng.st = final_state;
    }
  }
  if (by_progress) __builtin_amdgcn_s_setprio(0);

  if constexpr (CHUNKS) {
    if (chunk + 1u < n_chunks) {
      if (active) {
        auto st = [&](int wd, uint32_t v) { a.chunk_state[(size_t)wd * a.tile_pixels + tp] = v; };
        auto stf = [&](int wd, float v) { st(wd, __float_as_uint(v)); };
#pragma unroll
        for (int q = 0; q < kOwn; q++) {
          const int f = s * kOwn + q;
          if (f < 3) {
            stf(PT_REC_COLOR + 3 * f, sum0[q]); stf(PT_REC_COLOR + 3 * f + 1, sum1[q]); stf(PT_REC_COLOR + 3 * f + 2, sum2[q]);
          } else {
            stf(PT_REC_DEPTH, sum0[q]);
          }
          if (f < 2) st(PT_REC_N_COLOR + f, (uint32_t)w[q].n);
          stf(PT_REC_MEAN + 2 * f, w[q].mean);
          stf(PT_REC_M2 + 2 * f, w[q].M2);
        }
        if constexpr (RNG == PT_RNG_XORWOW) {
          if (s == 0) {
            st(PT_REC_RNG, final_state.d); st(PT_REC_RNG + 1, final_state.v0); st(PT_REC_RNG + 2, final_state.v1); st(PT_REC_RNG + 3, final_state.v2); st(PT_REC_RNG + 4, final_state.v3); st(PT_REC_RNG + 5, final_state.v4);
          }
        }
      }
      chunk_publish(a, block_id, chunk);
      return;
    }
  }

  if (active) {
    const float fs = (float)a.spp;
    const bool planar = !REF && a.planar;
    float* o = planar ? a.out + tp : a.out + (size_t)tp * 14;
    const size_t cs = planar ? (size_t)a.tile_pixels : 1;
#pragma unroll
    for (int q = 0; q < kOwn; q++) {
      const int f = s * kOwn + q;
      if (f < 3) {
        const float v0 = sum0[q] / fs, v1 = sum1[q] / fs, v2 = sum2[q] / fs;
        o[(3 * f + 0) * cs] = v0;
        o[(3 * f + 1) * cs] = v1;
        o[(3 * f + 2) * cs] = v2;
        if (f == 0 && a.vertices) store_display_vertex(a.vertices + (size_t)tp * 3, a.width, row, col, v0, v1, v2);
      } else {
        o[9 * cs] = sum0[q] / fs;
      }
      o[(10 + f) * cs] = welford_variance(w[q]);
    }
    if constexpr (RNG == PT_RNG_XORWOW) {
      if (a.rng_state && s == 0) {
        uint32_t* p = a.rng_state + (size_t)tp * 6;
        p[0] = final_state.d; p[1] = final_state.v0; p[2] = final_state.v1;
        p[3] = final_state.v2; p[4] = final_state.v3; p[5] = final_state.v4;
      }
    }
  }
  if constexpr (CHUNKS) {
    if (n_chunks > 1u) chunk_publish(a, block_id, chunk);
  }
}

__global__ void __launch_bounds__(PT_BLOCK_THREADS)
    setup_random_kernel(uint32_t* state, int width, int row_begin, uint32_t tile_pixels, uint64_t seed) {
  const uint32_t tp = blockIdx.x * PT_BLOCK_THREADS + threadIdx.x;
  if (tp >= tile_pixels) return;
  const uint32_t id = (uint32_t)(row_begin + (int)(tp / (uint32_t)width)) * (uint32_t)width + tp % (uint32_t)width;
  Xorwow s;
  xorwow_init(s, (uint64_t)id + seed);
  uint32_t* p = state + (size_t)tp * 6;
  p[0] = s.d;
  p[1] = s.v0;
  p[2] = s.v1;
  p[3] = s.v2;
  p[4] = s.v3;
  p[5] = s.v4;
}

}

#include <utility>

const VariantInfo& pt_kernel_variant(int variant) { return (variant >= 0 && variant < kNumVariants) ? kVariants[variant] : kNoVariant; }
int pt_kernel_num_variants(void) { return kNumVariants; }
int pt_kernel_block_threads(int variant) { return pt_kernel_variant(variant).threads; }
bool pt_kernel_has_variant(int variant) { return variant >= 0 && variant < kNumVariants && (PT_BUILD_EXPERIMENTS || kVariants[variant].product); }
bool pt_kernel_has_resume(int variant) { return pt_kernel_variant(variant).resume; }

static inline bool lds_lean(int n, const VariantInfo& v) { return v.lean == PT_LEAN_ALWAYS || (v.lean == PT_LEAN_BIG && n > PT_SCREEN_MAX_SPHERES); }
static inline size_t scene_lds_f4(int n, const VariantInfo& v) {
  if (lds_lean(n, v)) return pt::kTablesF4;
  return (size_t)n * 4 + pt::kTablesF4 +
         (v.lds_extra == PT_LDS_PACKED ? (size_t)((n + 1) / 2) * 2 : v.lds_extra == PT_LDS_WALLS ? (size_t)pt::kWallF4 : 0);
}
static inline size_t tail_lds_bytes(int n, const VariantInfo& v) {
  if (v.grid == PT_GRID_LANE) return n <= pt::kGridMaxSpheres ? pt::grid_lds_bytes(n, false) : 64;
  if (v.grid == PT_GRID_POOLED)
    return (n <= pt::kGridMaxSpheres ? ((pt::grid_lds_bytes(n, true, v.threads) + 15) & ~(size_t)15) : 64) + (v.threads / 64) * pt::kPoolWaveBytes;
  if (v.split()) return (PT_BLOCK_THREADS / 64) * 64 * pt::kRecWords * sizeof(float);
  return (PT_BLOCK_THREADS / 64) * 64 * 14 * sizeof(float);
}
static inline size_t scene_lds_bytes(int n, const VariantInfo& v) { return scene_lds_f4(n, v) * sizeof(float4) + tail_lds_bytes(n, v); }
size_t pt_kernel_lds_bytes(int n_spheres, int variant) { return scene_lds_bytes(n_spheres, pt_kernel_variant(variant)); }

static inline int ref_config(int n, int max_bounces, const VariantInfo& v, bool planar) {
  return (n == 9 && (max_bounces == 5 || max_bounces == 8) && !planar && v.ref_builds) ? max_bounces : 0;
}
int pt_kernel_ref_bounces(int n_spheres, int max_bounces, int variant, bool planar) { return ref_config(n_spheres, max_bounces, pt_kernel_variant(variant), planar); }

template <bool FRAMES, bool RESUME, bool ADAPTIVE>
using kernel_fn = void (*)(typename pt::KernelArgsOf<FRAMES, RESUME, ADAPTIVE>::type);

template <bool FRAMES, bool RESUME, bool ADAPTIVE, int RNG, int VAR, bool LEAN, int REFB>
static kernel_fn<FRAMES, RESUME, ADAPTIVE> kernel_build() {
  constexpr VariantInfo v = kVariants[VAR];
  if constexpr (v.split()) return pt::pixel_kernel_split<RNG, v.lanes, LEAN, REFB>;
  else return pt::pixel_kernel<RNG, v.kernel, LEAN, REFB, FRAMES, v.wide, RESUME, ADAPTIVE>;
}

template <bool FRAMES, bool RESUME, bool ADAPTIVE, int RNG, int VAR>
static kernel_fn<FRAMES, RESUME, ADAPTIVE> variant_kernel(bool lean, int ref) {
  constexpr VariantInfo v = kVariants[VAR];
  if constexpr ((v.product || PT_BUILD_EXPERIMENTS) && (!RESUME || v.resume) && (!FRAMES || v.frames)) {
    if constexpr (v.ref_builds) {
      if (ref == 5 && !lean) return kernel_build<FRAMES, RESUME, ADAPTIVE, RNG, VAR, false, 5>();
      if (ref == 8 && !lean) return kernel_build<FRAMES, RESUME, ADAPTIVE, RNG, VAR, false, 8>();
    }
    if constexpr (!FRAMES) {
      if constexpr (v.lean != PT_LEAN_NEVER) {
        if (lean) return kernel_build<FRAMES, RESUME, ADAPTIVE, RNG, VAR, true, 0>();
      }
      if constexpr (v.lean != PT_LEAN_ALWAYS) {
        if (!lean) return kernel_build<FRAMES, RESUME, ADAPTIVE, RNG, VAR, false, 0>();
      }
    }
  }
  return nullptr;
}

template <bool FRAMES, bool RESUME, bool ADAPTIVE, int RNG, int... VAR>
static kernel_fn<FRAMES, RESUME, ADAPTIVE> select_kernel_of(int variant, bool lean, int ref, std::integer_sequence<int, VAR...>) {
  static constexpr kernel_fn<FRAMES, RESUME, ADAPTIVE> (*of[])(bool, int) = {variant_kernel<FRAMES, RESUME, ADAPTIVE, RNG, VAR>...};
  return (variant >= 0 && variant < kNumVariants) ? of[variant](lean, ref) : nullptr;
}

static inline int run_variant(int variant, int max_bounces) { return (variant == 12 && max_bounces < 1) ? 11 : variant; }

template <bool FRAMES = false, bool RESUME = false, bool ADAPTIVE = false>
static kernel_fn<FRAMES, RESUME, ADAPTIVE> select_kernel(int rng_mode, int variant, int n_spheres, int max_bounces, bool planar) {
  const VariantInfo& v = pt_kernel_variant(variant);
  const bool lean = lds_lean(n_spheres, v);
  const int ref = ref_config(n_spheres, max_bounces, v, planar);
  const std::make_integer_sequence<int, kNumVariants> all;
  return rng_mode == PT_RNG_PHILOX ? select_kernel_of<FRAMES, RESUME, ADAPTIVE, PT_RNG_PHILOX>(variant, lean, ref, all)
                                   : select_kernel_of<FRAMES, RESUME, ADAPTIVE, PT_RNG_XORWOW>(variant, lean, ref, all);
}

const void* pt_kernel_symbol(int rng_mode, int variant, int n_spheres, int max_bounces, bool planar) {
  return (const void*)select_kernel<>(rng_mode, run_variant(variant, max_bounces), n_spheres, max_bounces, planar);
}
const void* pt_resume_kernel_symbol(int rng_mode, int variant, int n_spheres, int max_bounces, bool planar) {
  return (const void*)select_kernel<false, true>(rng_mode, variant, n_spheres, max_bounces, planar);
}
const void* pt_adaptive_kernel_symbol(int rng_mode, int variant, int n_spheres, int max_bounces, bool planar) {
  return (const void*)select_kernel<false, true, true>(rng_mode, variant, n_spheres, max_bounces, planar);
}

#ifdef PT_SCREEN_STATS
extern "C" int pt_debug_screen_stats(unsigned long long out[8], int reset) {
  unsigned long long zero[8] = {0, 0, 0, 0, 0, 0, 0, 0};
  if (hipMemcpyFromSymbol(out, HIP_SYMBOL(pt::g_screen_stats), sizeof(zero)) != hipSuccess) return -2;
  if (reset && hipMemcpyToSymbol(HIP_SYMBOL(pt::g_screen_stats), zero, sizeof(zero)) != hipSuccess) return -2;
  return 0;
}
#endif

#ifdef PT_GRID_STATS
extern "C" int pt_debug_grid_hist(unsigned long long out[256], int reset) {
  static unsigned long long zero[256];
  if (hipMemcpyFromSymbol(out, HIP_SYMBOL(pt::g_grid_hist), sizeof(zero)) != hipSuccess) return -2;
  if (reset && hipMemcpyToSymbol(HIP_SYMBOL(pt::g_grid_hist), zero, sizeof(zero)) != hipSuccess) return -2;
  return 0;
}
extern "C" int pt_debug_grid_stats(unsigned long long out[8], int reset) {
  unsigned long long zero[8] = {0, 0, 0, 0, 0, 0, 0, 0};
  if (hipMemcpyFromSymbol(out, HIP_SYMBOL(pt::g_grid_stats), sizeof(zero)) != hipSuccess) return -2;
  if (reset && hipMemcpyToSymbol(HIP_SYMBOL(pt::g_grid_stats), zero, sizeof(zero)) != hipSuccess) return -2;
  return 0;
}
#endif

size_t pt_kernel_accel_bytes(void) { return pt::kGridAccelBytes; }

int pt_kernel_max_spheres(int variant) {
  const VariantInfo& v = pt_kernel_variant(variant);
  if (v.lean != PT_LEAN_NEVER) return 1 << 26;
  const size_t fixed = tail_lds_bytes(0, v) + pt::kTablesF4 * sizeof(float4);
  if (v.lds_extra == PT_LDS_PACKED) return (int)((PT_LDS_BUDGET_BYTES - fixed - 2 * sizeof(float4)) / (5 * sizeof(float4)));
  return (int)((PT_LDS_BUDGET_BYTES - fixed) / (4 * sizeof(float4)));
}

hipError_t pt_launch_build_grid(const pt_sphere* spheres, int n, uint32_t* accel, const float* eye, bool pooled, hipStream_t stream, int threads) {
  hipLaunchKernelGGL(pt::build_grid_kernel, dim3(1), dim3(pt::kGridBuildThreads), 0, stream, spheres, n, accel, eye ? eye[0] : 0.0f,
                     eye ? eye[1] : 0.0f, eye ? eye[2] : 0.0f, eye ? 1 : 0, pt::grid_max_entries(n, pooled, threads));
  return hipGetLastError();
}

void pt_kernel_grid_layout(int n_spheres, int threads, uint64_t out[8]) {
  out[0] = pt::kGridAccelBytes;
  out[1] = pt::kGridBigOff;
  out[2] = pt::kGridStartOff;
  out[3] = pt::kGridItemsOff;
  out[4] = pt::kGridCellsOff;
  out[5] = pt::kGridEmisOff;
  out[6] = (uint64_t)pt::kGridMaxCells;
  out[7] = (uint64_t)pt::grid_max_entries(n_spheres, true, threads);
}

bool pt_kernel_chunked(int variant, int n_spheres, int max_bounces, bool planar, int spp, uint32_t chunks) {
  const VariantInfo& v = pt_kernel_variant(variant);
  const bool build_chunks = v.chunk_build(!lds_lean(n_spheres, v) && ref_config(n_spheres, max_bounces, v, planar));
  return build_chunks && chunks > 1u && chunks <= (uint32_t)PT_CHUNKS_MAX && spp >= 2 * (int)chunks &&
         (spp + (int)chunks - 1) / (int)chunks <= (v.chunk_family == PT_CHUNK_GRID ? PT_CHUNK_MAX_SAMPLES_GRID : PT_CHUNK_MAX_SAMPLES);
}

struct LaunchShape {
  unsigned block, blocks;
  size_t lds;
};
static hipError_t prepare_launch(const void* fn, const VariantInfo& v, PixelKernelArgs& b, int samples, hipStream_t stream, LaunchShape* s) {
  if (!fn) return hipErrorInvalidValue;
  b.scene_lds_f4 = (uint32_t)scene_lds_f4(b.n_spheres, v);
  b.prio = (samples >= PT_PRIO_MIN_SPP || b.prio != 0u) ? 1u : 0u;
  s->lds = scene_lds_bytes(b.n_spheres, v);
  const size_t lds_budget = v.wide ? (size_t)PT_LDS_WIDE_BUDGET_BYTES : (size_t)PT_LDS_BUDGET_BYTES;
  if (s->lds > lds_budget) return hipErrorInvalidValue;
  if (s->lds > 64 * 1024) {
    hipError_t e = hipFuncSetAttribute(fn, hipFuncAttributeMaxDynamicSharedMemorySize, (int)lds_budget);
    if (e != hipSuccess) return e;
  }
  if (v.grid != PT_GRID_NONE) {
    if (!b.accel) return hipErrorInvalidValue;
    hipError_t e = pt_launch_build_grid(b.spheres, b.n_spheres, const_cast<uint32_t*>(b.accel), b.eye, v.grid == PT_GRID_POOLED, stream, v.threads);
    if (e != hipSuccess) return e;
  }
  s->block = (unsigned)v.threads;
  s->blocks = (unsigned)(((uint64_t)b.tile_pixels * (uint64_t)v.lanes + s->block - 1) / s->block);
  return hipSuccess;
}

#if PT_BUILD_EXPERIMENTS
static inline uint32_t census_modes(const PixelKernelArgs& b, bool ref, int samples) {
  return (b.chunks > 1u ? PT_CENSUS_MODE_CHUNKED : 0u) | (b.repair != 0u ? PT_CENSUS_MODE_REPAIR : 0u) | (b.planar != 0u ? PT_CENSUS_MODE_PLANAR : 0u) |
         (b.vertices ? PT_CENSUS_MODE_VERTICES : 0u) | (b.rng_state ? PT_CENSUS_MODE_RNG_STATE : 0u) |
         (ref && samples >= PT_FOOTPRINT_MIN_SPP ? PT_CENSUS_MODE_FOOTPRINT : 0u) | (b.prio != 0u ? PT_CENSUS_MODE_PRIO : 0u);
}
#endif

hipError_t pt_launch_pixel_kernel(const PixelKernelArgs& a, int rng_mode, int variant, hipStream_t stream) {
  variant = run_variant(variant, a.max_bounces);
  const auto fn = select_kernel<>(rng_mode, variant, a.n_spheres, a.max_bounces, a.planar != 0u);
  PixelKernelArgs b = a;
  LaunchShape s;
  hipError_t e = prepare_launch((const void*)fn, pt_kernel_variant(variant), b, a.spp, stream, &s);
  if (e != hipSuccess) return e;
  const bool chunked = a.repair == 0u && pt_kernel_chunked(variant, a.n_spheres, a.max_bounces, a.planar != 0u, a.spp, a.chunks) && a.chunk_state && a.chunk_flag;
  if (a.repair != 0u && !a.chunk_flag) return hipErrorInvalidValue;
  b.chunks = chunked ? a.chunks : 0u;
  unsigned grid = s.blocks;
  if (chunked) {
    e = hipMemsetAsync(a.chunk_flag, 0, (size_t)grid * sizeof(uint32_t), stream);
    if (e != hipSuccess) return e;
    grid *= a.chunks;
  }
  hipLaunchKernelGGL(fn, dim3(grid), dim3(s.block), s.lds, stream, b);
  return PT_LAUNCHED(fn, census_modes(b, ref_config(a.n_spheres, a.max_bounces, pt_kernel_variant(variant), a.planar != 0u) != 0, a.spp));
}

bool pt_kernel_has_frames(int variant, int n_spheres, int max_bounces, bool planar) {
  const VariantInfo& v = pt_kernel_variant(variant);
  return v.frames && ref_config(n_spheres, max_bounces, v, planar) != 0;
}

hipError_t pt_launch_frames_kernel(const FramesKernelArgs& fa, int rng_mode, int variant, hipStream_t stream) {
  const PixelKernelArgs& a = fa.base;
  if (!pt_kernel_has_frames(variant, a.n_spheres, a.max_bounces, a.planar != 0u) || fa.frames < 2u || fa.frames > (uint32_t)PT_FRAMES_MAX) return hipErrorInvalidValue;
  const auto fn = select_kernel<true>(rng_mode, variant, a.n_spheres, a.max_bounces, a.planar != 0u);
  FramesKernelArgs b = fa;
  b.base.chunks = 0u;
  b.base.repair = 0u;
  LaunchShape s;
  const hipError_t e = prepare_launch((const void*)fn, pt_kernel_variant(variant), b.base, a.spp, stream, &s);
  if (e != hipSuccess) return e;
  hipLaunchKernelGGL(fn, dim3(rng_mode == PT_RNG_PHILOX ? s.blocks * fa.frames : s.blocks), dim3(s.block), s.lds, stream, b);
  return PT_LAUNCHED(fn, census_modes(b.base, true, a.spp));
}

hipError_t pt_launch_setup_random(uint32_t* state, int width, int row_begin, uint32_t tile_pixels, uint64_t seed,
                                  hipStream_t stream) {
  const unsigned grid = (tile_pixels + PT_BLOCK_THREADS - 1) / PT_BLOCK_THREADS;
  hipLaunchKernelGGL(pt::setup_random_kernel, dim3(grid), dim3(PT_BLOCK_THREADS), 0, stream, state, width, row_begin,
                     tile_pixels, seed);
  return hipGetLastError();
}

template <bool ADAPTIVE, class Args>
static hipError_t launch_pass(const Args& ra, int rng_mode, int variant, hipStream_t stream) {
  const PixelKernelArgs& a = ra.base;
  if (!pt_kernel_has_resume(variant) || !ra.session || ra.sample_begin < 0 || ra.sample_begin >= a.spp || a.rng_state) return hipErrorInvalidValue;
  const auto fn = select_kernel<false, true, ADAPTIVE>(rng_mode, variant, a.n_spheres, a.max_bounces, a.planar != 0u);
  Args b = ra;
  b.base.chunks = 0u;
  b.base.chunk_state = nullptr;
  b.base.chunk_flag = nullptr;
  b.base.repair = 0u;
  LaunchShape s;
  const hipError_t e = prepare_launch((const void*)fn, pt_kernel_variant(variant), b.base, a.spp - ra.sample_begin, stream, &s);
  if (e != hipSuccess) return e;
  hipLaunchKernelGGL(fn, dim3(s.blocks), dim3(s.block), s.lds, stream, b);
  return PT_LAUNCHED(fn, census_modes(b.base, ref_config(a.n_spheres, a.max_bounces, pt_kernel_variant(variant), a.planar != 0u) != 0, a.spp - ra.sample_begin) |
                             (ra.sample_begin == 0 ? (uint32_t)PT_CENSUS_MODE_FIRST_PASS : 0u));
}

hipError_t pt_launch_resume_kernel(const ResumeKernelArgs& ra, int rng_mode, int variant, hipStream_t stream) {
  return launch_pass<false>(ra, rng_mode, variant, stream);
}
// ... 118 lines not shown
```

### cuda-pathtrace_amd/csrc/pt_scene_lds.h

```cpp
#pragma once
#include "pt_device.h"
#include "pt_kernel.h"
#include "pt_walls.h"

#pragma clang fp contract(off)

namespace pt {

#define PT_PRAGMA_(x) _Pragma(#x)
#define PT_UNROLL(n) PT_PRAGMA_(unroll n)

struct GridLds;

struct SceneLds {
  float4* geom;
  float4* mat0;
  float4* mat1;
  float4* eyeg;
  float* inv1;
  double* rden1;
  float* rcpn;
  float4* pair;
  const pt_sphere* global;
  bool lean;
  bool small_only;
  const GridLds* grid;
  void* pool;
  uint32_t prim_mask;
  uint32_t absmask;
  const uint4* walls = nullptr;

  __device__ __forceinline__ float4 geom_uniform(int i) const {
    if (lean) {
      typedef float f4u __attribute__((ext_vector_type(4), aligned(4)));
      typedef const __attribute__((address_space(4))) f4u* cptr;
      typedef const __attribute__((address_space(4))) char* cbytes;
      const f4u v = *(cptr)((cbytes)global + (size_t)i * sizeof(pt_sphere));
      return make_float4(v.y, v.z, v.w, v.x * v.x);
    }
    return geom[i];
  }
  __device__ __forceinline__ float4 geom_lane(int i) const {
    if (lean) {
      const pt_sphere* sp = global + i;
      return make_float4(sp->pos[0], sp->pos[1], sp->pos[2], sp->radius * sp->radius);
    }
    return geom[i];
  }
};

typedef float v2f __attribute__((ext_vector_type(2)));

constexpr int kTablesF4 = kUnitTabSize / 4 + kUnitTabSize / 2 + (kRcpTab + 4) / 4;

template <bool WITH_PAIR>
__device__ __forceinline__ SceneLds stage_scene(const pt_sphere* __restrict__ spheres, int n, float4* lds, bool lean, F3 eye,
                                                int spp, bool lean_tables = true) {
  float4* tab = lean ? lds : lds + 4 * n;
  const bool tables = !lean | lean_tables;
  SceneLds s{lds, lds + n, lds + 2 * n, lds + 3 * n, tables ? reinterpret_cast<float*>(tab) : nullptr,
             tables ? reinterpret_cast<double*>(tab + kUnitTabSize / 4) : nullptr,
             tables ? reinterpret_cast<float*>(tab + kUnitTabSize / 4 + kUnitTabSize / 2) : nullptr, lds + 4 * n + kTablesF4,
             spheres, lean, false, nullptr, nullptr, 0xFFFFFFFFu, vgpr_const<0x7FFFFFFFu>()};
  const float qnan = __builtin_nanf("");
  if (tables) {
    for (int i = threadIdx.x; i < kUnitTabSize; i += blockDim.x)
      s.inv1[i] = 1.0f / sqrtf(__uint_as_float(0x3F800000u - (uint32_t)kUnitTabHalf + (uint32_t)i));
    for (int i = threadIdx.x; i < kUnitTabSize; i += blockDim.x) {
      const float a = __uint_as_float(0x3F800000u - (uint32_t)kUnitTabHalf + (uint32_t)i);
      s.rden1[i] = ray_const_rden(2.0 * (double)a);
    }
    const int counts = spp < kRcpTab ? spp : kRcpTab;
    for (int i = threadIdx.x; i < counts; i += blockDim.x) s.rcpn[i] = 1.0f / (float)(i + 1);
    if (threadIdx.x == 0) s.rcpn[kRcpTab] = qnan;
  }
  if (lean) {
    __syncthreads();
    return s;
  }
  for (int i = threadIdx.x; i < n; i += blockDim.x) {
    const pt_sphere sp = spheres[i];
    const float rr = sp.radius * sp.radius;
    s.geom[i] = make_float4(sp.pos[0], sp.pos[1], sp.pos[2], rr);
    s.mat0[i] = make_float4(sp.emission[0], sp.emission[1], sp.emission[2], sp.color[0]);
    s.mat1[i] = make_float4(sp.color[1], sp.color[2], luminance(mk3(sp.color[0], sp.color[1], sp.color[2])), 0.0f);
    const F3 off = mk3(eye.x - sp.pos[0], eye.y - sp.pos[1], eye.z - sp.pos[2]);
    s.eyeg[i] = make_float4(off.x, off.y, off.z, dot(off, off) - rr);
    if constexpr (WITH_PAIR) {
      float* pa = reinterpret_cast<float*>(s.pair + 2 * (i >> 1)) + (i & 1);
      pa[0] = sp.pos[0];
      pa[2] = sp.pos[1];
      pa[4] = sp.pos[2];
      pa[6] = rr;
      if ((i == n - 1) && !(i & 1)) {
        pa[1] = qnan;
        pa[3] = qnan;
        pa[5] = qnan;
        pa[7] = qnan;
      }
    }
  }
  __syncthreads();
  return s;
}

__device__ __forceinline__ uint32_t lds_addr(const void* p) {
  return (uint32_t)(uintptr_t)(const __attribute__((address_space(3))) char*)p;
}
__device__ __forceinline__ float4 lds_read_f4(uint32_t addr) {
  typedef float f4v __attribute__((ext_vector_type(4)));
  const f4v v = *(const __attribute__((address_space(3))) f4v*)(uintptr_t)addr;
  return make_float4(v.x, v.y, v.z, v.w);
}

constexpr int kWallF4 = 7;
__device__ __forceinline__ void stage_walls(SceneLds& s, const pt_sphere* __restrict__ spheres, int n) {
  uint4* W = reinterpret_cast<uint4*>(s.pair);
  if (threadIdx.x == 0) {
    const WallLayout w = classify_walls(spheres, n);
    for (int k = 0; k < 3; k++) {
      const float4 g = s.geom[w.obj[k]];
      W[k] = make_uint4(__float_as_uint(g.x), __float_as_uint(g.y), __float_as_uint(g.z), __float_as_uint(g.w));
      W[4 + k] = make_uint4(lds_addr(s.geom + w.minus[k]), lds_addr(s.geom + w.plus[k]), (uint32_t)w.minus[k], (uint32_t)w.plus[k]);
    }
    W[3] = make_uint4((uint32_t)w.obj[0], (uint32_t)w.obj[1], (uint32_t)w.obj[2], w.ok ? 0x3F802000u : 0x7F800000u);
  }
  __syncthreads();
  s.walls = W;
}

__device__ __forceinline__ void fetch_material(const SceneLds& sc, int idx, F3& emis, F3& scol, float* lum_col = nullptr) {
  if (sc.lean) {
#ifdef PT_TIMING_ONLY_NO_MATERIAL
    emis = mk3(0.0f, 0.0f, 0.0f);
    scol = mk3(0.5f, 0.5f, 0.5f);
    if (lum_col) *lum_col = 0.5f;
    return;
#endif
    const pt_sphere* sp = sc.global + idx;
    emis = mk3(sp->emission[0], sp->emission[1], sp->emission[2]);
    scol = mk3(sp->color[0], sp->color[1], sp->color[2]);
    if (lum_col) *lum_col = luminance(scol);
  } else {
    const float4 m0 = sc.mat0[idx];
    const float4 m1 = sc.mat1[idx];
    emis = mk3(m0.x, m0.y, m0.z);
    scol = mk3(m0.w, m1.x, m1.y);
    if (lum_col) *lum_col = m1.z;
  }
}

struct TraceOutput {
  F3 color, normal, albedo;
  float depth;
};

__device__ __forceinline__ void frame_values(const TraceOutput& L, const Welford var[4], float fs, float px[14]) {
  px[0] = L.color.x / fs;
  px[1] = L.color.y / fs;
  px[2] = L.color.z / fs;
  px[3] = L.normal.x / fs;
  px[4] = L.normal.y / fs;
  px[5] = L.normal.z / fs;
  px[6] = L.albedo.x / fs;
  px[7] = L.albedo.y / fs;
  px[8] = L.albedo.z / fs;
  px[9] = L.depth / fs;
  px[10] = welford_variance(var[0]);
  px[11] = welford_variance(var[1]);
  px[12] = welford_variance(var[2]);
  px[13] = welford_variance(var[3]);
}

template <int RNG>
struct Rng;

template <>
struct Rng<PT_RNG_XORWOW> {
  Xorwow st;
  __device__ __forceinline__ void begin_sample(uint32_t) {}
  __device__ __forceinline__ void jitter(float& jx, float& jy) {
    jx = uniform_from_u32(xorwow_next(st));
    jy = uniform_from_u32(xorwow_next(st));
  }
  __device__ __forceinline__ void bounce(int, float& az, float& el) {
    az = uniform_from_u32(xorwow_next(st));
    el = uniform_from_u32(xorwow_next(st));
  }
};

template <>
struct Rng<PT_RNG_PHILOX> {
  uint32_t k0, k1, pix, sample;
  uint4 blk;
  __device__ __forceinline__ void begin_sample(uint32_t s) {
    sample = s;
    blk = philox4x32_10(make_uint4(pix, sample, 0u, 0u), k0, k1);
  }
  __device__ __forceinline__ void jitter(float& jx, float& jy) {
    jx = uniform_from_u32(blk.x);
    jy = uniform_from_u32(blk.y);
  }
  __device__ __forceinline__ void bounce(int n, float& az, float& el) {
    if (n & 1) blk = philox4x32_10(make_uint4(pix, sample, (uint32_t)((n + 1) >> 1), 0u), k0, k1);
    bool second = (n == 0) || (((n + 1) & 1) != 0);
    az = uniform_from_u32(second ? blk.z : blk.x);
    el = uniform_from_u32(second ? blk.w : blk.y);
  }
};

}
// ... 1 lines not shown
```

### cuda-pathtrace_amd/csrc/pt_walls.h

```cpp
#pragma once
#include <math.h>
#include "../../include/ptcore.h"

namespace pt {

struct WallLayout {
  int obj[3];
  int minus[3];
  int plus[3];
  bool ok;
};

__host__ __device__ inline WallLayout classify_walls(const pt_sphere* s, int n) {
  WallLayout w{{6, 7, 8}, {0, 2, 4}, {1, 3, 5}, false};
  const WallLayout none = w;
  if (n != 9) return w;
  double rmax = 0.0;
  for (int i = 0; i < 9; i++) {
    const double r = (double)s[i].radius;
    if (!(r >= 0.0) || !(r < 1e30)) return none;
    rmax = r > rmax ? r : rmax;
  }
  int walls[6], objs[3], nw = 0, no = 0;
  for (int i = 0; i < 9; i++) {
    if ((double)s[i].radius >= 0.5 * rmax) {
      if (nw == 6) return none;
      walls[nw++] = i;
    } else {
      if (no == 3) return none;
      objs[no++] = i;
    }
  }
  if (nw != 6 || no != 3) return none;
  double p[3] = {0.0, 0.0, 0.0};
  for (int j = 0; j < 6; j++)
    for (int k = 0; k < 3; k++) p[k] += (double)s[walls[j]].pos[k] / 6.0;
  double ext = 0.0;
  for (int j = 0; j < 3; j++)
    for (int k = 0; k < 3; k++) {
      const double e = fabs((double)s[objs[j]].pos[k] - p[k]);
      if (!(e < 1e30)) return none;
      ext = e > ext ? e : ext;
    }
  int mi[3] = {-1, -1, -1}, pl[3] = {-1, -1, -1};
  for (int j = 0; j < 6; j++) {
    const pt_sphere& sw = s[walls[j]];
    const double r = (double)sw.radius;
    if (sw.emission[0] != 0.0f || sw.emission[1] != 0.0f || sw.emission[2] != 0.0f) return none;
    if (!(r >= 100.0 * ext) || !(r > 0.0)) return none;
    double off[3];
    int ax = 0;
    for (int k = 0; k < 3; k++) {
      off[k] = (double)sw.pos[k] - p[k];
      if (!(fabs(off[k]) < 1e30)) return none;
      if (fabs(off[k]) > fabs(off[ax])) ax = k;
    }
    if (!(fabs(off[ax]) >= 0.5 * r)) return none;
    for (int k = 0; k < 3; k++)
      if (k != ax && !(fabs(off[k]) <= 1e-2 * r)) return none;
    int* slot = off[ax] > 0.0 ? &pl[ax] : &mi[ax];
    if (*slot >= 0) return none;
    *slot = walls[j];
  }
  for (int k = 0; k < 3; k++) {
    if (mi[k] < 0 || pl[k] < 0) return none;
    const pt_sphere &a = s[pl[k]], &b = s[mi[k]];
    if (!((double)a.pos[k] - (double)a.radius < (double)b.pos[k] + (double)b.radius)) return none;
    for (int j = 0; j < 3; j++)
      if (j != k && __builtin_bit_cast(unsigned, a.pos[j]) != __builtin_bit_cast(unsigned, b.pos[j])) return none;
  }
  for (int k = 0; k < 3; k++) {
    w.obj[k] = objs[k];
    w.minus[k] = mi[k];
    w.plus[k] = pl[k];
  }
  w.ok = true;
  return w;
}

}
```

### include/ptcore_lab.h

```cpp
#ifndef PTCORE_LAB_H
#define PTCORE_LAB_H

#include "ptcore.h"

#ifdef __cplusplus
extern "C" {
#endif

enum {
  PT_FN_INV_SQRT_LITERAL = 0,
  PT_FN_INV_SQRT_FAST = 1,
  PT_FN_SQRT_LITERAL = 2,
  PT_FN_SQRT_FAST = 3,
  PT_FN_SIN = 4,
  PT_FN_COS = 5,
  PT_FN_UNIFORM = 6,
  PT_FN_ONEMINUS_LITERAL = 7,
  PT_FN_ONEMINUS_FAST = 8,
  PT_FN_ONEMINUS_F32 = 9,
  PT_FN_ONEMINUS_F32_FLAG = 10,
  PT_FN_ZERO = 11,
  PT_FN_UNIFORM_LITERAL = 12,
  PT_FN_SIN_LITERAL = 13,
  PT_FN_COS_LITERAL = 14,
  PT_FN_COUNT = 15
};
int pt_debug_unary_map(int fn, const float* d_in, float* d_out, size_t n);
int pt_debug_unary_compare(int fn_a, int fn_b, uint32_t first_bits, uint64_t count, uint64_t* n_mismatch,
                           uint32_t* example_bits);
int pt_debug_div_compare(uint32_t n_first, uint32_t n_count, uint32_t first_bits, uint64_t count, uint64_t* n_mismatch,
                         uint32_t* example_bits, uint32_t* example_n);
int pt_debug_grid_header(const pt_sphere* d_spheres, int n_spheres, uint32_t header_out[16]);
int pt_debug_grid_image(const pt_sphere* d_spheres, int n_spheres, const float* eye, int threads, uint32_t* image_out,
                        size_t image_bytes, uint64_t layout_out[8]);
int pt_debug_policy_ms(int rng_mode, int variant, double waves_per_simd, int spp, int bounces, double* ms);
int pt_debug_policy_choice(int rng_mode, double waves_per_simd, int spp, int bounces, int with9, int chunked, int* variant);
int pt_debug_renderer_batch_launches(pt_renderer* r, uint32_t* launches);

#define PT_BUILD_INFO_WORDS 8
int pt_debug_kernel_builds(int index, int* n_builds, int32_t info[PT_BUILD_INFO_WORDS]);
#define PT_ROW_INFO_WORDS 12
int pt_debug_variant_row(int row, int* n_rows, int32_t info[PT_ROW_INFO_WORDS]);
enum {
  PT_CENSUS_MODE_CHUNKED = 1,
  PT_CENSUS_MODE_REPAIR = 2,
  PT_CENSUS_MODE_PLANAR = 4,
  PT_CENSUS_MODE_VERTICES = 8,
  PT_CENSUS_MODE_RNG_STATE = 16,
  PT_CENSUS_MODE_FOOTPRINT = 32,
  PT_CENSUS_MODE_FIRST_PASS = 64,
  PT_CENSUS_MODE_PRIO = 128
};
int pt_debug_launch_census(int index, uint32_t* launches, uint32_t* modes);
int pt_debug_launch_census_reset(void);

int pt_debug_fast_nearest(const pt_sphere* d_spheres, int n_spheres, const float* d_rays, uint32_t n_rays, int specialised, int last,
                          uint32_t mask, float* d_t, int32_t* d_idx);

int pt_debug_denoiser_layer_info(pt_denoiser* d, int layer, int* n_layers, int shape[3], char* name, size_t name_len);
int pt_debug_denoiser_activation(pt_denoiser* d, int layer, float* h_out, size_t n_floats);
int pt_debug_denoiser_set_activation(pt_denoiser* d, int layer, const float* h_in, size_t n_floats);
int pt_debug_denoiser_activation_frames(pt_denoiser* d, int layer, int frames, float* h_out, size_t n_floats);
int pt_debug_denoiser_set_activation_frames(pt_denoiser* d, int layer, int frames, const float* h_in, size_t n_floats);
int pt_debug_denoiser_conv_info(pt_denoiser* d, int conv, int* n_convs, int info[12], char* name, size_t name_len);
int pt_debug_denoiser_run_conv(pt_denoiser* d, int conv, float* d_rgb);
int pt_debug_denoiser_run_conv_frames(pt_denoiser* d, int conv, float* d_out, int frames, int ld, size_t frame_stride);
int pt_debug_denoiser_run_pre(pt_denoiser* d, float* d_frames, int frames, size_t frame_stride, int inplace);
int pt_debug_denoiser_memory(pt_denoiser* d, int layer, uint64_t info[6]);
int pt_debug_denoiser_last_enqueue(pt_denoiser* d, int* groups, int* launches);
int pt_debug_denoiser_conv_plan(pt_denoiser* d, int n_frames, int conv, int info[6]);

int pt_debug_filter_step(pt_filter* f, float* d_frame, float* d_rgb, int samples, const uint32_t* d_counts, int step);
int pt_debug_filter_tiled(pt_filter* f, int on);
int pt_debug_filter_state(pt_filter* f, const float* d_frame, int samples, const uint32_t* d_counts, const int* steps, int n_steps,
                          float* d_state, float* d_guide0, float* d_guide1);

int pt_debug_progressive_set_samples(pt_progressive* p, int64_t samples);
int pt_debug_progressive_record(pt_progressive* p, uint32_t* host);
int pt_debug_progressive_set_active(pt_progressive* p, const uint8_t* host_mask);
int pt_debug_adaptive_select(const uint32_t* rec, uint32_t tile_pixels, int width, int n, int n_end, int mode, int peek,
                             const pt_adaptive_opts* opts, uint8_t* mask, uint32_t* counts, uint32_t* list, uint32_t words[2],
                             uint32_t* block_sums);
int pt_debug_adaptive_finalize(const uint32_t* rec, const uint32_t* counts, uint32_t tile_pixels, int planar, float* out);

#ifdef __cplusplus
}
#endif
#endif
```

Before: 24700.

## Precompute wall classification and share cross-axis wall terms in screening

Wall classification moves out of the per-block kernel prologue into a one-thread pre-kernel that writes a small record, which blocks read to stage walls in parallel across three threads. When the record says the wall spheres share coordinates across axes, a specialised sample loop reuses squared and product terms between the three wall pairs and hard-codes the certification scale. This removes redundant per-ray arithmetic in the nine-sphere wall screen and the serial per-block classification. In exchange it adds a kernel launch per render, duplicates the sample loop, and adds optional debug counters in experiment builds.

```diff
diff --git a/cuda-pathtrace_amd/__init__.py b/cuda-pathtrace_amd/__init__.py
--- a/cuda-pathtrace_amd/__init__.py
+++ b/cuda-pathtrace_amd/__init__.py
@@ -235,6 +235,7 @@
     "pt_debug_policy_ms": (ctypes.c_int, [ctypes.c_int, ctypes.c_int, ctypes.c_double, ctypes.c_int, ctypes.c_int, ctypes.POINTER(ctypes.c_double)]),
     "pt_debug_policy_choice": (ctypes.c_int, [ctypes.c_int, ctypes.c_double, ctypes.c_int, ctypes.c_int, ctypes.c_int, ctypes.c_int, ctypes.POINTER(ctypes.c_int)]),
     "pt_debug_renderer_batch_launches": (ctypes.c_int, [_vp, ctypes.POINTER(ctypes.c_uint32)]),
+    "pt_debug_renderer_wall_stats": (ctypes.c_int, [_vp, ctypes.c_int, ctypes.POINTER(ctypes.c_uint64)]),
     "pt_debug_kernel_builds": (ctypes.c_int, [ctypes.c_int, ctypes.POINTER(ctypes.c_int), ctypes.POINTER(ctypes.c_int32)]),
     "pt_debug_variant_row": (ctypes.c_int, [ctypes.c_int, ctypes.POINTER(ctypes.c_int), ctypes.POINTER(ctypes.c_int32)]),
     "pt_debug_launch_census": (ctypes.c_int, [ctypes.c_int, ctypes.POINTER(ctypes.c_uint32), ctypes.POINTER(ctypes.c_uint32)]),
@@ -679,6 +680,14 @@
         check(lib.pt_debug_renderer_batch_launches(self.handle, ctypes.byref(n)))
         return n.value
 
+    def wall_stats(self, on=None):
+        if on is not None:
+            check(self._lab("pt_debug_renderer_wall_stats")(self.handle, 1 if on else 2, None))
+            return None
+        out = (ctypes.c_uint64 * 4)()
+        check(self._lab("pt_debug_renderer_wall_stats")(self.handle, 0, out))
+        return tuple(int(v) for v in out)
+
     def kernel_info(self, n_spheres):
         ki = KernelInfo()
         check(lib.pt_renderer_kernel_info(self.handle, n_spheres, ctypes.byref(ki)))
diff --git a/cuda-pathtrace_amd/csrc/pt_capi.hip b/cuda-pathtrace_amd/csrc/pt_capi.hip
--- a/cuda-pathtrace_amd/csrc/pt_capi.hip
+++ b/cuda-pathtrace_amd/csrc/pt_capi.hip
@@ -10,6 +10,7 @@
 
 #include "pt_internal.h"
 #include "pt_kernel.h"
+#include "pt_walls.h"
 
 namespace {
 thread_local char g_err[512] = "";
@@ -42,6 +43,7 @@
   hipEvent_t ev_fail = nullptr;
   bool fail_pending = false;
   uint32_t* d_accel = nullptr;
+  uint32_t* d_walls = nullptr;
   uint32_t* d_chunk = nullptr;
   uint32_t chunks[PT_CHUNK_FAMILIES] = {};
   uint64_t chunk_wait_ticks = 0;
@@ -319,6 +321,8 @@
   if (e == hipSuccess) e = hipHostMalloc((void**)&r->h_fail, sizeof(uint32_t), hipHostMallocDefault);
   if (e == hipSuccess) { *r->h_fail = 0; e = hipEventCreateWithFlags(&r->ev_fail, hipEventDisableTiming); }
   if (e == hipSuccess) e = hipMalloc((void**)&r->d_accel, pt_kernel_accel_bytes());
+  if (e == hipSuccess) e = hipMalloc((void**)&r->d_walls, pt_kernel_wall_bytes());
+  if (e == hipSuccess) e = hipMemset(r->d_walls, 0, pt_kernel_wall_bytes());
   if (e == hipSuccess) {
     set_chunk_counts(r, prop);
     int khz = 0;
@@ -359,6 +363,7 @@
   if (!r) return PT_OK;
   if (r->d_state) (void)hipFree(r->d_state);
   if (r->d_accel) (void)hipFree(r->d_accel);
+  if (r->d_walls) (void)hipFree(r->d_walls);
   if (r->d_chunk) (void)hipFree(r->d_chunk);
   if (r->d_err) (void)hipFree(r->d_err);
   if (r->h_err) (void)hipHostFree(r->h_err);
@@ -422,7 +427,7 @@
     return pt_fail(PT_ELIMIT, "render: %d spheres exceed the LDS staging limit of %d", n_spheres,
                    pt_kernel_max_spheres(variant));
   a->fail_count = r->d_fail;
-  a->accel = r->d_accel;
+  a->accel = pt_kernel_reads_walls(variant, n_spheres, r->opts.max_bounces, r->opts.layout == PT_LAYOUT_PLANAR) ? r->d_walls : r->d_accel;
   a->scene_lds_f4 = 0;
   a->planar = r->opts.layout == PT_LAYOUT_PLANAR ? 1u : 0u;
   r->launch_variant = variant;
@@ -564,6 +569,20 @@
   *launches = r->batch_launches;
   return PT_OK;
 }
+
+int pt_debug_renderer_wall_stats(pt_renderer* r, int mode, uint64_t out[4]) {
+  if (!r || mode < 0 || mode > 2 || (mode == 0 && !out)) return pt_fail(PT_EINVAL, "pt_debug_renderer_wall_stats: bad arguments");
+  PT_HIP(hipSetDevice(r->device));
+  PT_HIP(hipDeviceSynchronize());
+  char* stats = reinterpret_cast<char*>(r->d_walls) + pt::kWallStatsOffset;
+  if (mode == 0) {
+    PT_HIP(hipMemcpy(out, stats, 4 * sizeof(uint64_t), hipMemcpyDeviceToHost));
+  } else {
+    PT_HIP(hipMemset(stats, 0, 4 * sizeof(uint64_t)));
+    r->debug = mode == 1 ? (r->debug | PT_DEBUG_WALL_STATS) : (r->debug & ~PT_DEBUG_WALL_STATS);
+  }
+  return PT_OK;
+}
 #endif
 
 int pt_renderer_render(pt_renderer* r, float* d_out, const pt_sphere* d_spheres, int n_spheres, const float basis[12],
@@ -742,7 +761,7 @@
   a.frame = 0u;
   a.planar = r->opts.layout == PT_LAYOUT_PLANAR ? 1u : 0u;
   a.fail_count = nullptr;
-  a.accel = r->d_accel;
+  a.accel = pt_kernel_reads_walls(v, n_spheres, r->opts.max_bounces, r->opts.layout == PT_LAYOUT_PLANAR) ? r->d_walls : r->d_accel;
   a.seed = r->opts.seed;
   a.err_word = r->d_err;
   a.chunk_wait_ticks = r->chunk_wait_ticks;
diff --git a/cuda-pathtrace_amd/csrc/pt_intersect.h b/cuda-pathtrace_amd/csrc/pt_intersect.h
--- a/cuda-pathtrace_amd/csrc/pt_intersect.h
+++ b/cuda-pathtrace_amd/csrc/pt_intersect.h
@@ -157,6 +157,7 @@
 };
 
 __device__ __forceinline__ uint32_t screen_sphere_oc(F3 off, float c, int i, F3 d, const RayConst& rc, uint32_t imask, ScreenState& st);
+__device__ __forceinline__ uint32_t screen_sphere_hc(float h, float c, int i, const RayConst& rc, uint32_t imask, ScreenState& st);
 __device__ __forceinline__ uint32_t screen_sphere(const float4 g, int i, F3 o, F3 d, const RayConst& rc, uint32_t imask,
                                                   ScreenState& st) {
   const F3 off = mk3(o.x - g.x, o.y - g.y, o.z - g.z);
@@ -183,7 +184,9 @@
   st.k2 = umin(umin(umax(l, lead[2]), r2), next[2]);
 }
 __device__ __forceinline__ uint32_t screen_sphere_oc(F3 off, float c, int i, F3 d, const RayConst& rc, uint32_t imask, ScreenState& st) {
-  const float h = dot(d, off);
+  return screen_sphere_hc(dot(d, off), c, i, rc, imask, st);
+}
+__device__ __forceinline__ uint32_t screen_sphere_hc(float h, float c, int i, const RayConst& rc, uint32_t imask, ScreenState& st) {
   const float hh = h * h;
   const float ac = rc.a * c;
   const float dacc = fmaf(-rc.a, c, hh);
@@ -206,21 +209,52 @@
 __device__ __forceinline__ F3 with_axis(F3 v, float x) {
   return mk3(AX == 0 ? x : v.x, AX == 1 ? x : v.y, AX == 2 ? x : v.z);
 }
-template <int AX>
+struct WallTerms {
+  F3 sq, pr;
+};
+template <int AX, int C>
+constexpr bool kWallTermFresh = AX == 0 || C == AX || (AX == 1 && C == 0);
+template <int AX, bool SHARE>
 __device__ __forceinline__ uint32_t screen_wall_pair(const uint4 t, uint32_t m, F3 o, F3 d, const RayConst& rc, uint32_t imask,
-                                                     ScreenState& st, float& hb, bool& inb) {
+                                                     ScreenState& st, float& hb, bool& inb, WallTerms& sh) {
   const float4 gf = lds_read_f4(bitop3<0xE4>(t.y, t.x, m)), gb = lds_read_f4(bitop3<0xE4>(t.x, t.y, m));
-  const F3 off = mk3(o.x - gf.x, o.y - gf.y, o.z - gf.z);
-  const F3 sq = off * off, pr = d * off;
   const float ob = AX == 0 ? o.x - gb.x : AX == 1 ? o.y - gb.y : o.z - gb.z;
-  const F3 sqb = with_axis<AX>(sq, ob * ob), prb = with_axis<AX>(pr, (AX == 0 ? d.x : AX == 1 ? d.y : d.z) * ob);
-  hb = (prb.x + prb.y) + prb.z;
-  inb = neg_finite(fmaf(gb.w, 5.9837103e-08f, ((sqb.x + sqb.y) + sqb.z) - gb.w));
-  return screen_sphere_oc(off, ((sq.x + sq.y) + sq.z) - gf.w, (int)bitop3<0xE4>(t.w, t.z, m), d, rc, imask, st);
-}
-template <bool WALLS>
+  const float db = AX == 0 ? d.x : AX == 1 ? d.y : d.z;
+  if constexpr (SHARE) {
+    F3 sq = sh.sq, pr = sh.pr;
+    if constexpr (kWallTermFresh<AX, 0>) {
+      const float f = o.x - gf.x;
+      sq.x = f * f;
+      pr.x = d.x * f;
+    }
+    if constexpr (kWallTermFresh<AX, 1>) {
+      const float f = o.y - gf.y;
+      sq.y = f * f;
+      pr.y = d.y * f;
+    }
+    if constexpr (kWallTermFresh<AX, 2>) {
+      const float f = o.z - gf.z;
+      sq.z = f * f;
+      pr.z = d.z * f;
+    }
+    sh.sq = with_axis<AX>(sq, AX == 0 ? sh.sq.x : AX == 1 ? sh.sq.y : sh.sq.z);
+    sh.pr = with_axis<AX>(pr, AX == 0 ? sh.pr.x : AX == 1 ? sh.pr.y : sh.pr.z);
+    const F3 sqb = with_axis<AX>(sq, ob * ob), prb = with_axis<AX>(pr, db * ob);
+    hb = (prb.x + prb.y) + prb.z;
+    inb = neg_finite(fmaf(gb.w, 5.9837103e-08f, ((sqb.x + sqb.y) + sqb.z) - gb.w));
+    return screen_sphere_hc((pr.x + pr.y) + pr.z, ((sq.x + sq.y) + sq.z) - gf.w, (int)bitop3<0xE4>(t.w, t.z, m), rc, imask, st);
+  } else {
+    const F3 off = mk3(o.x - gf.x, o.y - gf.y, o.z - gf.z);
+    const F3 sq = off * off, pr = d * off;
+    const F3 sqb = with_axis<AX>(sq, ob * ob), prb = with_axis<AX>(pr, db * ob);
+    hb = (prb.x + prb.y) + prb.z;
+    inb = neg_finite(fmaf(gb.w, 5.9837103e-08f, ((sqb.x + sqb.y) + sqb.z) - gb.w));
+    return screen_sphere_oc(off, ((sq.x + sq.y) + sq.z) - gf.w, (int)bitop3<0xE4>(t.w, t.z, m), d, rc, imask, st);
+  }
+}
+template <bool ASSUME>
 __device__ __forceinline__ void screen_walled(ScreenState& st, const uint4* W, F3 o, F3 d, const RayConst& rc, uint32_t imask,
-                                              uint32_t lim_hi_bits) {
+                                              uint32_t lim_hi_bits, unsigned long long* stats = nullptr) {
   auto umin = [](uint32_t x, uint32_t y) { return x < y ? x : y; };
   auto umax = [](uint32_t x, uint32_t y) { return x > y ? x : y; };
   const float4* Wg = reinterpret_cast<const float4*>(W);
@@ -232,20 +266,28 @@
   const uint32_t l0 = umin(umin(a0, a1), a2), n0 = umed3(a0, a1, a2);
   float h0, h1, h2;
   bool in0, in1, in2;
-  if constexpr (WALLS) __builtin_amdgcn_sched_barrier(0);
-  const uint32_t b0 = screen_wall_pair<0>(W[4], mx, o, d, rc, imask, st, h0, in0);
-  if constexpr (WALLS) __builtin_amdgcn_sched_barrier(0);
-  const uint32_t b1 = screen_wall_pair<1>(W[5], my, o, d, rc, imask, st, h1, in1);
-  if constexpr (WALLS) __builtin_amdgcn_sched_barrier(0);
-  const uint32_t b2 = screen_wall_pair<2>(W[6], mz, o, d, rc, imask, st, h2, in2);
-  if constexpr (WALLS) __builtin_amdgcn_sched_barrier(0);
+  WallTerms sh{mk3(0.0f, 0.0f, 0.0f), mk3(0.0f, 0.0f, 0.0f)};
+  if constexpr (ASSUME) __builtin_amdgcn_sched_barrier(0);
+  const uint32_t b0 = screen_wall_pair<0, ASSUME>(W[4], mx, o, d, rc, imask, st, h0, in0, sh);
+  if constexpr (ASSUME) __builtin_amdgcn_sched_barrier(0);
+  const uint32_t b1 = screen_wall_pair<1, ASSUME>(W[5], my, o, d, rc, imask, st, h1, in1, sh);
+  if constexpr (ASSUME) __builtin_amdgcn_sched_barrier(0);
+  const uint32_t b2 = screen_wall_pair<2, ASSUME>(W[6], mz, o, d, rc, imask, st, h2, in2, sh);
+  if constexpr (ASSUME) __builtin_amdgcn_sched_barrier(0);
   const uint32_t l1 = umin(umin(b0, b1), b2), n1 = umed3(b0, b1, b2);
   st.k1 = umin(l0, l1);
   st.k2 = umin(umin(umax(l0, l1), n0), n1);
-  const float K = __uint_as_float(st.k1 & ~imask) * __uint_as_float(oi.w);
+  const float K = __uint_as_float(st.k1 & ~imask) * (ASSUME ? 1.0009765625f : __uint_as_float(oi.w));
   const bool cert = (st.k1 < lim_hi_bits) & (neg_finite(fmaf(2.0f, h0, K)) & in0) & (neg_finite(fmaf(2.0f, h1, K)) & in1) &
                     (neg_finite(fmaf(2.0f, h2, K)) & in2);
-  if (__builtin_expect(__builtin_amdgcn_ballot_w64(!cert) != 0, 0)) {
+  const bool fallback = __builtin_amdgcn_ballot_w64(!cert) != 0;
+#if PT_BUILD_EXPERIMENTS
+  if (stats && __builtin_amdgcn_mbcnt_hi(~0u, __builtin_amdgcn_mbcnt_lo(~0u, 0u)) == 0u) {
+    atomicAdd(stats + 2, 1ull);
+    if (fallback) atomicAdd(stats + 3, 1ull);
+  }
+#endif
+  if (__builtin_expect(fallback, 0)) {
     auto behind = [&](int k, uint32_t m) {
       const uint4 t = W[4 + k];
       screen_insert(st, screen_sphere(lds_read_f4(bitop3<0xE4>(t.x, t.y, m)), (int)bitop3<0xE4>(t.z, t.w, m), o, d, rc, imask, st));
@@ -294,7 +336,11 @@
 #if PT_UNROLL_NINE
   if constexpr (!PRIMARY) {
     if (sc.walls && n == 9) {
+#if PT_BUILD_EXPERIMENTS
+      screen_walled<WALLS>(st, sc.walls, o, d, rc, imask, lim_hi_bits, sc.wall_stats);
+#else
       screen_walled<WALLS>(st, sc.walls, o, d, rc, imask, lim_hi_bits);
+#endif
       i = 9;
     }
   }
diff --git a/cuda-pathtrace_amd/csrc/pt_kernel.h b/cuda-pathtrace_amd/csrc/pt_kernel.h
--- a/cuda-pathtrace_amd/csrc/pt_kernel.h
+++ b/cuda-pathtrace_amd/csrc/pt_kernel.h
@@ -148,6 +148,7 @@
 #define PT_DEVERR_CHUNK_CHAIN 1u
 #define PT_CHUNK_FAILED 0x80000000u
 #define PT_DEBUG_DROP_CHUNK_FLAG 1u
+#define PT_DEBUG_WALL_STATS 2u
 
 #ifndef PT_BUILD_EXPERIMENTS
 #define PT_BUILD_EXPERIMENTS 0
@@ -183,6 +184,8 @@
 int pt_kernel_num_variants(void);
 bool pt_kernel_chunked(int variant, int n_spheres, int max_bounces, bool planar, int spp, uint32_t chunks);
 int pt_kernel_ref_bounces(int n_spheres, int max_bounces, int variant, bool planar);
+bool pt_kernel_reads_walls(int variant, int n_spheres, int max_bounces, bool planar);
+size_t pt_kernel_wall_bytes(void);
 int pt_kernel_block_threads(int variant);
 bool pt_kernel_has_variant(int variant);
 const void* pt_kernel_symbol(int rng_mode, int variant, int n_spheres, int max_bounces, bool planar);
diff --git a/cuda-pathtrace_amd/csrc/pt_kernel.hip b/cuda-pathtrace_amd/csrc/pt_kernel.hip
--- a/cuda-pathtrace_amd/csrc/pt_kernel.hip
+++ b/cuda-pathtrace_amd/csrc/pt_kernel.hip
@@ -1,3 +1,5 @@
+#include <type_traits>
+
 #include "pt_trace.h"
 
 #pragma clang fp contract(off)
@@ -156,7 +158,18 @@
   SceneLds sc = stage_scene<K.lds_extra == PT_LDS_PACKED>(a.spheres, a.n_spheres, lds_scene, LEAN, mk3(a.eye[0], a.eye[1], a.eye[2]), a.spp);
   sc.small_only = !LEAN && K.lean == PT_LEAN_BIG;
   constexpr bool kWalls = K.lds_extra == PT_LDS_WALLS && REFB == 5 && !LEAN;
-  if constexpr (kWalls) stage_walls(sc, a.spheres, a.n_spheres);
+  bool assume = false;
+  if constexpr (kWalls) {
+    assume = __builtin_amdgcn_readfirstlane(a.accel[3]) != 0u;
+    if (assume) stage_walls(sc, a.accel);
+#if PT_BUILD_EXPERIMENTS
+    if (a.debug & PT_DEBUG_WALL_STATS) {
+      unsigned long long* stats = reinterpret_cast<unsigned long long*>(const_cast<uint32_t*>(a.accel) + kWallStatsOffset / 4);
+      if (threadIdx.x == 0) atomicAdd(stats + (assume ? 0 : 1), 1ull);
+      sc.wall_stats = stats;
+    }
+#endif
+  }
   constexpr bool kRegen = K.loop == PT_LOOP_REGEN, kDecoupled = K.loop == PT_LOOP_DECOUPLED;
   GridLds grid;
   if constexpr (K.grid != PT_GRID_NONE) {
@@ -460,6 +473,30 @@
     const int q1 = i_begin + span / 4, q2 = i_begin + span / 2, q3 = i_end - span / 4;
     const int stride_mask = span >= 64 ? 15 : 0;
     const int i_stop = active ? i_end : i;
+    if constexpr (kWalls) {
+      auto sample_loop = [&](auto assume_c, const SceneLds& s) __attribute__((always_inline)) {
+        constexpr bool ASSUME = decltype(assume_c)::value;
+        for (; i < i_stop; i++) {
+          if (by_progress) {
+            const int iu = __builtin_amdgcn_readfirstlane(i);
+            if ((iu & stride_mask) == 0) {
+              if (iu < q1) __builtin_amdgcn_s_setprio(3);
+              else if (iu < q2) __builtin_amdgcn_s_setprio(2);
+              else if (iu < q3) __builtin_amdgcn_s_setprio(1);
+              else __builtin_amdgcn_s_setprio(0);
+            }
+          }
+          rng.begin_sample((uint32_t)i);
+          F3 dir;
+          primary_ray(rng, dir);
+          trace_ray<RNG, K.tracer, REFB, ASSUME>(L, s, a.n_spheres, eye, dir, rng, var, a.max_bounces);
+        }
+      };
+      if (__builtin_expect(!assume, 0)) sample_loop(std::false_type{}, sc);
+      SceneLds scw = sc;
+      scw.walls = wall_block(sc);
+      sample_loop(std::true_type{}, scw);
+    } else {
     for (; i < i_stop; i++) {
       if (by_progress) {
         const int iu = __builtin_amdgcn_readfirstlane(i);
@@ -473,7 +510,8 @@
       rng.begin_sample((uint32_t)i);
       F3 dir;
       primary_ray(rng, dir);
-      trace_ray<RNG, K.tracer, REFB, kWalls>(L, sc, a.n_spheres, eye, dir, rng, var, a.max_bounces);
+      trace_ray<RNG, K.tracer, REFB>(L, sc, a.n_spheres, eye, dir, rng, var, a.max_bounces);
+    }
     }
     if (by_progress) __builtin_amdgcn_s_setprio(0);
   }
@@ -916,6 +954,14 @@
   p[5] = s.v4;
 }
 
+__global__ void __launch_bounds__(64) classify_walls_kernel(const pt_sphere* __restrict__ spheres, int n, uint32_t* __restrict__ rec) {
+  if (threadIdx.x != 0 || blockIdx.x != 0) return;
+  unsigned r[kWallRecordWords];
+  wall_record(spheres, n, r);
+#pragma unroll
+  for (int k = 0; k < kWallRecordWords; k++) rec[k] = r[k];
+}
+
 }
 
 #include <utility>
@@ -945,6 +991,11 @@
 static inline int ref_config(int n, int max_bounces, const VariantInfo& v, bool planar) {
   return (n == 9 && (max_bounces == 5 || max_bounces == 8) && !planar && v.ref_builds) ? max_bounces : 0;
 }
+static inline bool wall_build(int n, int max_bounces, const VariantInfo& v, bool planar) {
+  return v.lds_extra == PT_LDS_WALLS && !v.split() && !lds_lean(n, v) && ref_config(n, max_bounces, v, planar) == 5;
+}
+bool pt_kernel_reads_walls(int variant, int n_spheres, int max_bounces, bool planar) { return wall_build(n_spheres, max_bounces, pt_kernel_variant(variant), planar); }
+size_t pt_kernel_wall_bytes(void) { return pt::kWallBufferBytes; }
 int pt_kernel_ref_bounces(int n_spheres, int max_bounces, int variant, bool planar) { return ref_config(n_spheres, max_bounces, pt_kernel_variant(variant), planar); }
 
 template <bool FRAMES, bool RESUME, bool ADAPTIVE>
@@ -1081,6 +1132,12 @@
   if (v.grid != PT_GRID_NONE) {
     if (!b.accel) return hipErrorInvalidValue;
     hipError_t e = pt_launch_build_grid(b.spheres, b.n_spheres, const_cast<uint32_t*>(b.accel), b.eye, v.grid == PT_GRID_POOLED, stream, v.threads);
+    if (e != hipSuccess) return e;
+  }
+  if (wall_build(b.n_spheres, b.max_bounces, v, b.planar != 0u)) {
+    if (!b.accel) return hipErrorInvalidValue;
+    hipLaunchKernelGGL(pt::classify_walls_kernel, dim3(1), dim3(64), 0, stream, b.spheres, b.n_spheres, const_cast<uint32_t*>(b.accel));
+    const hipError_t e = hipGetLastError();
     if (e != hipSuccess) return e;
   }
   s->block = (unsigned)v.threads;
diff --git a/cuda-pathtrace_amd/csrc/pt_scene_lds.h b/cuda-pathtrace_amd/csrc/pt_scene_lds.h
--- a/cuda-pathtrace_amd/csrc/pt_scene_lds.h
+++ b/cuda-pathtrace_amd/csrc/pt_scene_lds.h
@@ -29,6 +29,9 @@
   uint32_t prim_mask;
   uint32_t absmask;
   const uint4* walls = nullptr;
+#if PT_BUILD_EXPERIMENTS
+  unsigned long long* wall_stats = nullptr;
+#endif
 
   __device__ __forceinline__ float4 geom_uniform(int i) const {
     if (lean) {
@@ -114,19 +117,18 @@
 }
 
 constexpr int kWallF4 = 7;
-__device__ __forceinline__ void stage_walls(SceneLds& s, const pt_sphere* __restrict__ spheres, int n) {
+__device__ __forceinline__ const uint4* wall_block(const SceneLds& s) { return reinterpret_cast<const uint4*>(s.pair); }
+__device__ __forceinline__ void stage_walls(const SceneLds& s, const uint32_t* __restrict__ rec) {
   uint4* W = reinterpret_cast<uint4*>(s.pair);
-  if (threadIdx.x == 0) {
-    const WallLayout w = classify_walls(spheres, n);
-    for (int k = 0; k < 3; k++) {
-      const float4 g = s.geom[w.obj[k]];
-      W[k] = make_uint4(__float_as_uint(g.x), __float_as_uint(g.y), __float_as_uint(g.z), __float_as_uint(g.w));
-      W[4 + k] = make_uint4(lds_addr(s.geom + w.minus[k]), lds_addr(s.geom + w.plus[k]), (uint32_t)w.minus[k], (uint32_t)w.plus[k]);
-    }
-    W[3] = make_uint4((uint32_t)w.obj[0], (uint32_t)w.obj[1], (uint32_t)w.obj[2], w.ok ? 0x3F802000u : 0x7F800000u);
+  if (threadIdx.x < 3) {
+    const int k = threadIdx.x;
+    const uint32_t obj = rec[k], mi = rec[4 + k], pl = rec[8 + k];
+    const float4 g = s.geom[obj];
+    W[k] = make_uint4(__float_as_uint(g.x), __float_as_uint(g.y), __float_as_uint(g.z), __float_as_uint(g.w));
+    W[4 + k] = make_uint4(lds_addr(s.geom + mi), lds_addr(s.geom + pl), mi, pl);
+    if (k == 0) W[3] = make_uint4(rec[0], rec[1], rec[2], 0u);
   }
   __syncthreads();
-  s.walls = W;
 }
 
 __device__ __forceinline__ void fetch_material(const SceneLds& sc, int idx, F3& emis, F3& scol, float* lum_col = nullptr) {
diff --git a/cuda-pathtrace_amd/csrc/pt_walls.h b/cuda-pathtrace_amd/csrc/pt_walls.h
--- a/cuda-pathtrace_amd/csrc/pt_walls.h
+++ b/cuda-pathtrace_amd/csrc/pt_walls.h
@@ -78,4 +78,24 @@
   return w;
 }
 
+__host__ __device__ inline bool walls_share_across_axes(const pt_sphere* s, const WallLayout& w) {
+  if (!w.ok) return false;
+  auto bits = [](float x) { return __builtin_bit_cast(unsigned, x); };
+  const pt_sphere &x = s[w.minus[0]], &y = s[w.minus[1]], &z = s[w.minus[2]];
+  return bits(y.pos[0]) == bits(z.pos[0]) && bits(x.pos[1]) == bits(z.pos[1]) && bits(x.pos[2]) == bits(y.pos[2]);
 }
+
+constexpr int kWallRecordWords = 12;
+constexpr int kWallStatsOffset = 64, kWallBufferBytes = 128;
+__host__ __device__ inline void wall_record(const pt_sphere* s, int n, unsigned rec[kWallRecordWords]) {
+  const WallLayout w = classify_walls(s, n);
+  for (int k = 0; k < 3; k++) {
+    rec[k] = (unsigned)w.obj[k];
+    rec[4 + k] = (unsigned)w.minus[k];
+    rec[8 + k] = (unsigned)w.plus[k];
+  }
+  rec[3] = walls_share_across_axes(s, w) ? 1u : 0u;
+  rec[7] = rec[11] = 0u;
+}
+
+}
diff --git a/include/ptcore_lab.h b/include/ptcore_lab.h
--- a/include/ptcore_lab.h
+++ b/include/ptcore_lab.h
@@ -36,6 +36,8 @@
 int pt_debug_policy_ms(int rng_mode, int variant, double waves_per_simd, int spp, int bounces, double* ms);
 int pt_debug_policy_choice(int rng_mode, double waves_per_simd, int spp, int bounces, int with9, int chunked, int* variant);
 int pt_debug_renderer_batch_launches(pt_renderer* r, uint32_t* launches);
+
+int pt_debug_renderer_wall_stats(pt_renderer* r, int mode, uint64_t out[4]);
 
 #define PT_BUILD_INFO_WORDS 8
 int pt_debug_kernel_builds(int index, int* n_builds, int32_t info[PT_BUILD_INFO_WORDS]);
```

After: 24900, median of 6. Within noise of the previous version (+0.8%).
